# wsntxxn/AudioCaption

Measured on AMD Instinct MI355X. Metric: clips/sec (10 s @ 32 kHz) encode+greedy-decode, Cnn14_Rnn-Trm, higher is better.
Workload: dtype bf16x3

## Files before the change

audiocaption_amd/_lib.py:

```python
import ctypes
import os

import torch

_HERE = os.path.dirname(os.path.abspath(__file__))
LIB_PATH = os.environ.get("AUDIOCAPTION_HIP_LIB") or os.path.join(_HERE, "libaudiocaption_hip.so")

AC_MAX_LAYERS = 8
AC_ENS_MAX = 8
ABI_VERSION = 2

c_float_p = ctypes.c_void_p
c_int_p = ctypes.c_void_p


class AcTrmLayer(ctypes.Structure):
    _fields_ = [(n, ctypes.c_void_p) for n in (
        "sa_in_w", "sa_in_b", "sa_out_w", "sa_out_b", "ca_in_w", "ca_in_b", "ca_out_w", "ca_out_b",
        "l1_w", "l1_b", "l2_w", "l2_b", "n1_w", "n1_b", "n2_w", "n2_b", "n3_w", "n3_b")]


class AcTrmWeights(ctypes.Structure):
    _fields_ = [(n, ctypes.c_int32) for n in (
        "d_model", "nhead", "nlayers", "dim_ff", "vocab", "max_pos", "attn_emb_dim", "reserved")] + [
        (n, ctypes.c_void_p) for n in ("emb", "pe", "cls_w", "proj_w", "proj_b", "proj_ln_w", "proj_ln_b", "step_pk")] + [
        ("layer", AcTrmLayer * AC_MAX_LAYERS)]


class AcTrmKeyword(ctypes.Structure):
    _fields_ = [("kwp", ctypes.c_void_p), ("ln_w", ctypes.c_void_p), ("ln_b", ctypes.c_void_p), ("row_div", ctypes.c_int32)]


class AcLogitRules(ctypes.Structure):
    _fields_ = [("repetition_penalty", ctypes.c_float), ("no_repeat_ngram", ctypes.c_int32), ("min_length", ctypes.c_int32),
                ("end_idx", ctypes.c_int32), ("n_bad", ctypes.c_int32), ("bad_words", ctypes.c_void_p)]


class AcBahWeights(ctypes.Structure):
    _fields_ = [(n, ctypes.c_int32) for n in (
        "emb_dim", "d_model", "attn_size", "attn_emb_dim", "fc_emb_dim", "vocab", "n_tags", "variant")] + [
        (n, ctypes.c_void_p) for n in ("emb", "temb", "w_ih", "w_hh", "b_ih", "b_hh", "attn_w", "attn_b", "attn_v",
                                       "fc_w", "fc_b", "ctx_w", "ctx_b", "cls_w", "cls_b")]


class AcBahGrads(ctypes.Structure):
    _fields_ = [(n, ctypes.c_void_p) for n in ("emb", "temb", "w_ih", "w_hh", "b_ih", "b_hh", "attn_w", "attn_b", "attn_v",
                                               "fc_w", "fc_b", "ctx_w", "ctx_b", "cls_w", "cls_b")]


_I, _L, _F, _P = ctypes.c_int, ctypes.c_long, ctypes.c_float, ctypes.c_void_p
_U64 = ctypes.c_ulonglong
_WP = ctypes.POINTER(AcTrmWeights)
_BP = ctypes.c_void_p

SIGNATURES = {
    "ac_abi_version": (_I, []),
    "ac_logmel": (_I, [_P, _I, _I, _I, _I, _P, _P, _P, _P, _P, _P, _P, _P, _I, _L, _L, _L, _P]),
    "ac_conv3x3_bn_relu": (_I, [_P, _P, _P, _P, _P, _I, _I, _I, _I, _I, _I, _I, _I, _P]),
    "ac_conv3x3_bn_relu_winograd": (_I, [_P, _P, _P, _P, _P, _I, _I, _I, _I, _I, _I, _I, _I, _P]),
    "ac_conv3x3_bn_relu_bf16x3": (_I, [_P, _P, _P, _P, _P, _I, _I, _I, _I, _I, _I, _I, _I, _P]),
    "ac_conv3x3_bn_relu_bf16x3_gw": (_I, [_P, _P, _P, _P, _P, _I, _I, _I, _I, _I, _I, _I, _I, _P]),
    "ac_conv3x3_bn_relu_wino1d": (_I, [_P, _P, _P, _P, _P, _I, _I, _I, _I, _I, _I, _I, _I, _P, _I, _I, _P]),
    "ac_conv3x3_bn_relu_wino1d_drop": (_I, [_P, _P, _P, _P, _P, _I, _I, _I, _I, _I, _I, _I, _I, _F, _U64, _P, _P]),
    "ac_conv3x3_wino1d_splitk_floats": (_L, [_I, _I, _I, _I, _I]),
    "ac_conv3x3_bn_relu_wino1d_splitk": (_I, [_P, _P, _P, _P, _P, _I, _I, _I, _I, _I, _I, _I, _I, _P, _I, _I, _P, _L, _P]),
    "ac_conv3x3_bn_relu_wino43": (_I, [_P, _P, _P, _P, _P, _I, _I, _I, _I, _I, _I, _I, _I, _I, _P, _I, _I, _P]),
    "ac_conv3x3_bn_relu_wino43_drop": (_I, [_P, _P, _P, _P, _P, _I, _I, _I, _I, _I, _I, _I, _I, _F, _U64, _P, _P]),
    "ac_conv3x3_wino43_workgroups": (_L, [_I, _I, _I, _I]),
    "ac_conv3x3_block1_wino43": (_I, [_P, _P, _P, _P, _P, _P, _P, _P, _I, _I, _I, _P, _I, _I, _F, _U64, _P, _P]),
    "ac_conv3x3_block1_wino43_mfma": (_I, [_P, _P, _P, _P, _P, _P, _P, _P, _I, _I, _I, _P, _I, _I, _F, _U64, _P, _P]),
    "ac_conv3x3_block1_conv2_wino43": (_I, [_P, _P, _P, _P, _P, _I, _I, _I, _P]),
    "ac_conv3x3_bn_relu_f16x2_gw": (_I, [_P, _P, _P, _P, _P, _I, _I, _I, _I, _I, _I, _I, _I, _I, _P, _P]),
    "ac_conv3x3_block1_f16x2": (_I, [_P, _P, _P, _P, _P, _P, _P, _P, _I, _I, _I, _I, _P, _P]),
    "ac_linear_bf16x3": (_I, [_P, _P, _P, _P, _P, _I, _I, _I, _I, _P]),
    "ac_conv3x3_first": (_I, [_P, _P, _P, _P, _P, _I, _I, _I, _I, _P]),
    "ac_conv3x3_first_f16": (_I, [_P, _P, _P, _P, _P, _I, _I, _I, _I, _P, _P]),
    "ac_conv5x5_first": (_I, [_P, _P, _P, _P, _P, _I, _I, _I, _P]),
    "ac_conv5x5_bn_relu_bf16x3": (_I, [_P, _P, _P, _P, _P, _I, _I, _I, _I, _I, _I, _I, _P]),
    "ac_pack_conv5x5_weight_bf16x3": (_I, [_P, _P, _I, _I, _P]),
    "ac_linear": (_I, [_P, _P, _P, _P, _I, _I, _I, _L, _L, _L, _I, _P]),
    "ac_gru_pack_whh": (_I, [_P, _P, _I, _P]),
    "ac_gru_layer": (_I, [_P, _P, _P, _P, _P, _I, _I, _I, _P]),
    "ac_gru_split_workspace_bytes": (_L, [_I]),
    "ac_gru_layer_split": (_I, [_P, _P, _P, _P, _P, _P, _P, _I, _I, _I, _P]),
    "ac_mean_with_lens": (_I, [_P, _P, _P, _I, _I, _I, _I, _P]),
    "ac_add_layernorm": (_I, [_P, _P, _P, _P, _P, _I, _I, _L, _L, _L, _P]),
    "ac_trm_memory": (_I, [_WP, _P, _I, _I, _P, _P, _P]),
    "ac_trm_step_pack_floats": (_L, [_WP]),
    "ac_trm_pack_step_weights": (_I, [_WP, _P, _P]),
    "ac_dec_wide_packed_floats": (_L, [_I, _I]),
    "ac_dec_wide_pack": (_I, [_P, _L, _I, _I, _P, _P]),
    "ac_dec_wide_gemm": (_I, [_I, _P, _L, _P, _L, _P, _P, _P, _L, _I, _P, _P, _F, _P, _L, _P, _P, _P, _L, _I, _I, _I, _I, _I, _I, _P]),
    "ac_trm_workspace_floats": (_L, [_WP, _I, _I]),
    "ac_trm_greedy": (_I, [_WP, _P, _P, _I, _I, _I, _I, _I, _I, _P, _P, _P, _P, _P, _P, _P]),
    "ac_trm_greedy_segments": (_I, [_WP, _P, _P, _I, _I, _I, _I, _I, _I, _I, _P, _P, _P, _P, _P, _P, _P]),
    "ac_sample_rows": (_I, [_P, _L, _I, _I, _I, _I, _F, _F, _P, _I, _P, _P, _P]),
    "ac_trm_sample": (_I, [_WP, _P, _P, _I, _I, _I, _I, _I, _I, _P, _P, _P, _P, _P, _P, _I, _I, _F, _F, _P, _P]),
    "ac_trm_sample_multi": (_I, [_WP, _P, _P, _I, _I, _I, _I, _I, _I, _I, _P, _P, _P, _P, _P, _P, _I, _I, _F, _F, _P, _P]),
    "ac_conv3x3_skinny_workspace_floats": (_L, [_I, _I, _I, _I, _I]),
    "ac_conv3x3_bn_relu_skinny": (_I, [_P, _P, _P, _P, _P, _I, _I, _I, _I, _I, _I, _I, _P, _L, _F, _U64, _P, _P]),
    "ac_trm_cluster_pack_floats": (_L, [_WP]),
    "ac_trm_cluster_pack": (_I, [_WP, _P, _P]),
    "ac_trm_cluster_workspace_bytes": (_L, [_I]),
    "ac_trm_greedy_cluster": (_I, [_WP, _P, _P, _P, _I, _I, _I, _I, _I, _I, _P, _P, _P, _P, _P, _P, _I, _P]),
    "ac_trm_forward_tokens": (_I, [_WP, _P, _P, _I, _I, _P, _P, _I, _P, _P, _P, _P]),
    "ac_trm_beam_step": (_I, [_WP, _P, _P, _I, _I, _I, _I, _I, _F, _P, _P, _P, _P, _P, _P, _P]),
    "ac_trm_beam_update": (_I, [_P, _P, _P, _P, _P, _P, _P, _P, _P, _P, _P, _P, _I, _I, _I, _I, _I, _I, _I, _I, _P]),
    "ac_trm_beam_reorder": (_I, [_WP, _I, _I, _I, _P, _P, _P]),
    "ac_trm_beam_update_all": (_I, [_P, _P, _P, _P, _P, _P, _P, _P, _P, _P, _P, _P, _I, _I, _I, _I, _I, _I, _I, _I, _P]),
    "ac_trm_kw_greedy_segments": (_I, [_WP, _P, _P, _P, _I, _I, _I, _I, _I, _I, _I, _P, _P, _P, _P, _P, _P, _P]),
    "ac_trm_kw_sample": (_I, [_WP, _P, _P, _P, _I, _I, _I, _I, _I, _I, _P, _P, _P, _P, _P, _P, _I, _I, _F, _F, _P, _P]),
    "ac_trm_kw_forward_tokens": (_I, [_WP, _P, _P, _P, _I, _I, _P, _P, _I, _P, _P, _P, _P]),
    "ac_trm_kw_beam_step": (_I, [_WP, _P, _P, _P, _I, _I, _I, _I, _I, _F, _P, _P, _P, _P, _P, _P, _P]),
    "ac_trm_kw_embed_qkv": (_I, [_WP, _P, _I, _I, _I, _P, _L, _P, _P, _P]),
    "ac_trm_step_logits": (_I, [_WP, _P, _P, _I, _I, _I, _I, _I, _P, _P, _I, _P, _L, _P, _L, _P, _P]),
    "ac_ens_greedy_pick": (_I, [_P, _I, _L, _I, _I, _I, _I, _I, _I, _P, _P, _P, _P, _P, _P, _P]),
    "ac_ens_sample_pick": (_I, [_P, _I, _L, _I, _I, _I, _I, _F, _F, _P, _I, _I, _I, _I, _P, _P, _P, _P, _P, _P, _P, _P]),
    "ac_ens_beam_step_select": (_I, [_P, _I, _L, _I, _I, _I, _I, _F, _P, _P, _P, _P, _P]),
    "ac_group_beam_select": (_I, [_P, _L, _I, _I, _I, _I, _F, _F, _P, _P, _I, _L, _P, _P, _P, _P]),
    "ac_logit_rules_apply": (_I, [_P, _L, _P, _L, _I, _I, _P, _L, _I, _P, _P]),
    "ac_trm_search_rules": (_I, [_WP, _P, _P, _I, _I, _I, _I, _I, _I, _I, _P, _P, _P, _P, _P, _P, _I, _I, _F, _F, _P, _P, _P, _L,
                                 _P]),
    "ac_trm_beam_step_rules": (_I, [_WP, _P, _P, _I, _I, _I, _I, _I, _F, _P, _P, _P, _P, _P, _P, _P, _P, _P]),
    "ac_bah_workspace_floats": (_L, [_BP, _I, _I, _I, _I]),
    "ac_bah_memory": (_I, [_BP, _P, _P, _I, _I, _I, _I, _P, _P]),
    "ac_bah_memory_cond": (_I, [_BP, _P, _P, _I, _I, _I, _I, _P, _P]),
    "ac_bah_step_logits": (_I, [_BP, _P, _P, _I, _I, _I, _I, _I, _P, _P, _L, _P, _P, _P, _L, _P, _L, _P, _L, _L, _P, _P]),
    "ac_bah_greedy": (_I, [_BP, _P, _P, _P, _I, _I, _I, _I, _I, _I, _P, _P, _P, _P, _P, _P, _P, _P, _P]),
    "ac_bah_sample": (_I, [_BP, _P, _P, _P, _I, _I, _I, _I, _I, _I, _P, _P, _P, _P, _P, _P, _P, _P, _I, _I, _F, _F, _P, _P]),
    "ac_bah_beam_gather": (_I, [_P, _P, _P, _P, _P, _P, _P, _I, _I, _I, _I, _I, _I, _P]),
    "ac_bah_train_workspace_floats": (_L, [_BP, _I, _I, _I]),
    "ac_bah_train_forward": (_I, [_BP, _P, _P, _P, _P, _L, _P, _P, _I, _I, _I, _I, _F, _U64, _P, _P, _P, _P, _P, _P, _P, _P,
                                  _P]),
    "ac_bah_train_rollout": (_I, [_BP, _P, _P, _P, _P, _I, _I, _I, _I, _I, _F, _P, _P, _L, _F, _U64, _P, _P, _P, _P, _P, _P, _P,
                                  _P, _P, _P]),
    "ac_bah_train_backward": (_I, [_BP, _P, _P, _P, _P, _P, _I, _I, _I, _F, _U64, _P, _P, _P, _P, _P]),
    "ac_bah_train_forward_cond": (_I, [_BP, _P, _P, _P, _P, _L, _P, _I, _I, _I, _I, _F, _U64, _P, _P, _P, _P, _P, _P, _P, _P,
                                       _P]),
    "ac_bah_train_backward_cond": (_I, [_BP, _P, _P, _P, _P, _P, _I, _I, _I, _F, _U64, _P, _P, _P, _P, _P]),
    "ac_bah_mean_lens_bwd": (_I, [_P, _P, _P, _I, _I, _I, _I, _P]),
    "ac_specificity_loss": (_I, [_P, _P, _P, _P, _I, _I, _I, _I, _P, _P, _P, _P, _P]),
    "ac_specificity_loss_bwd": (_I, [_P, _P, _P, _P, _P, _P, _P, _I, _I, _I, _I, _P, _P]),
    "ac_pool_avgmax": (_I, [_P, _P, _I, _I, _I, _I, _I, _I, _I, _I, _P]),
    "ac_sed_head": (_I, [_P, _P, _P, _P, _L, _I, _P]),
    "ac_sed_tag_workspace_bytes": (_L, [_I, _I, _I]),
    "ac_sed_temporal_tag": (_I, [_P, _I, _I, _I, _I, _I, _F, _F, _I, _P, _P, _L, _P, _P]),
    "ac_gemm": (_I, [_P, _L, _L, _P, _L, _L, _P, _L, _I, _I, _I, _P, _I, _F, _I, _F, _U64, _P, _L, _P, _I, _P]),
    "ac_gemm_bf16x3": (_I, [_P, _L, _L, _P, _L, _L, _P, _L, _I, _I, _I, _P, _I, _F, _I, _F, _U64, _P, _L, _P, _I, _P]),
    "ac_dropout": (_I, [_P, _P, _L, _F, _U64, _P, _L, _P]),
    "ac_mask_pos_scale": (_I, [_P, _P, _L, _F, _P]),
    "ac_build_prefix": (_I, [_P, _I, _P, _I, _P, _I, _I, _P, _L, _I, _I, _P]),
    "ac_embed_fwd": (_I, [_P, _P, _P, _P, _P, _L, _L, _I, _F, _U64, _F, _U64, _P, _P]),
    "ac_embed_bwd": (_I, [_P, _P, _P, _L, _I, _F, _U64, _F, _U64, _P, _P]),
    "ac_kw_embed_fwd": (_I, [_P, _P, _P, _P, _P, _P, _P, _P, _P, _P, _L, _L, _I, _F, _U64, _F, _U64, _P, _F, _P]),
    "ac_kw_embed_bwd": (_I, [_P, _P, _P, _P, _P, _P, _P, _P, _P, _L, _I, _F, _U64, _F, _U64, _P, _F, _P]),
    "ac_dropadd_ln_fwd": (_I, [_P, _P, _P, _P, _P, _P, _L, _L, _L, _I, _F, _U64, _P, _F, _P]),
    "ac_dropadd_ln_bwd": (_I, [_P, _P, _P, _P, _P, _I, _P, _L, _P, _P, _L, _I, _F, _U64, _P, _F, _P]),
    "ac_attn_seq_fwd": (_I, [_P, _L, _P, _L, _P, _L, _P, _L, _P, _I, _I, _P, _P, _P, _P, _P, _P, _I, _I, _I, _I, _I,
                             _I, _I, _I, _F, _U64, _P, _P]),
    "ac_attn_seq_bwd": (_I, [_P, _L, _P, _L, _P, _L, _P, _I, _I, _P, _L, _P, _L, _P, _L, _P, _L, _P, _P, _P, _P, _I,
                             _I, _I, _I, _I, _I, _F, _U64, _P, _P]),
    "ac_attn_self_bwd_tiled": (_I, [_P, _L, _P, _L, _P, _L, _P, _I, _I, _P, _L, _P, _L, _P, _L, _P, _L, _P, _P, _P, _P,
                                    _I, _I, _I, _I, _I, _I, _F, _U64, _P, _P, _P]),
    "ac_gather_rows": (_I, [_P, _P, _P, _L, _I, _P]),
    "ac_scatter_add_rows": (_I, [_P, _P, _P, _L, _I, _P]),
    "ac_specaug": (_I, [_P, _P, _P, _I, _I, _I, _I, _I, _I, _P]),
    "ac_sum_replicas": (_I, [_P, _P, _L, _I, _P]),
    "ac_rows_mean_w": (_I, [_P, _P, _I, _I, _I, _I, _I, _P]),
    "ac_transpose": (_I, [_P, _P, _I, _I, _I, _P]),
    "ac_colsum": (_I, [_P, _L, _P, _L, _I, _P]),
    "ac_argmax_rows": (_I, [_P, _L, _I, _I, _P, _L, _P]),
    "ac_label_smoothing_loss": (_I, [_P, _P, _L, _P, _I, _I, _I, _F, _F, _P, _P, _P, _F, _P, _P]),
    "ac_scst_pick": (_I, [_P, _L, _I, _I, _F, _P, _I, _I, _P, _L, _P, _P, _P, _L, _P, _L, _P]),
    "ac_scst_loss": (_I, [_P, _P, _L, _P, _F, _I, _I, _I, _I, _P, _P, _P, _P, _P]),
    "ac_scst_group_reward": (_I, [_P, _I, _I, _I, _P, _P, _P]),
    "ac_kd_loss": (_I, [_P, _P, _P, _L, _P, _I, _I, _I, _F, _F, _F, _F, _P, _P, _P, _P, _F, _P, _P]),
    "ac_enc_kd_workspace_floats": (_L, [_I, _I]),
    "ac_enc_kd_loss": (_I, [_P, _L, _P, _L, _I, _I, _I, _P, _P, _P, _P, _P, _F, _P, _P, _P]),
    "ac_cider_workspace_bytes": (_L, [_L, _I, _I, _I]),
    "ac_cider_scores": (_I, [_P, _I, _L, _I, _I, _I, _I, _P, _I, _I, _P, _L, _P, _I, _I, _P, _I, _P, _P, _I, _F, _P, _L, _P,
                             _P, _P]),
    "ac_capmetrics_workspace_bytes": (_L, [_I, _I]),
    "ac_bleu_scores": (_I, [_P, _I, _L, _I, _I, _I, _I, _P, _I, _P, _L, _P, _I, _I, _P, _I, _P, _P, _I, _P, _L, _P, _P, _P,
                            _P]),
    "ac_rouge_l_scores": (_I, [_P, _I, _L, _I, _I, _I, _I, _P, _I, _P, _L, _P, _I, _I, _P, _I, _P, _P, _P, _L, _P, _P, _P,
                               _P]),
    "ac_diversity_workspace_bytes": (_L, [_I, _I]),
    "ac_diversity_scores": (_I, [_P, _L, _I, _I, _I, _I, _P, _I, _P, _L, _P, _P, _P, _P, _P, _P]),
    "ac_diversity_group_workspace_bytes": (_L, [_I, _I, _I]),
    "ac_diversity_group_scores": (_I, [_P, _L, _I, _I, _I, _I, _P, _I, _P, _I, _P, _L, _P, _P, _P, _P, _P, _P, _P, _P]),
    "ac_gru_layer_train": (_I, [_P, _P, _P, _P, _P, _P, _I, _I, _I, _P]),
    "ac_gru_layer_bwd": (_I, [_P, _P, _P, _P, _P, _P, _P, _P, _I, _I, _I, _P]),
    "ac_swa_update": (_I, [_P, _P, _L, _I, _P]),
    "ac_grad_sumsq": (_I, [_P, _L, _P, _P]),
    "ac_clip_coef": (_I, [_P, _F, _F, _P]),
    "ac_scale_by_coef": (_I, [_P, _L, _P, _P]),
    "ac_adam_step": (_I, [_P, _P, _P, _P, _L, _P, _F, _F, _F, _F, _F, _I, _P, _P]),
    "ac_adam_commit": (_I, [_P, _P, _P]),
    "ac_pointwise_conv": (_I, [_P, _P, _P, _P, _L, _I, _I, _I, _F, _P, _I, _P]),
    "ac_top_db_clamp": (_I, [_P, _L, _F, _P, _I, _P]),
    "ac_effnet_stem": (_I, [_P, _P, _P, _P, _P, _I, _I, _I, _I, _I, _I, _P]),
    "ac_effnet_depthwise": (_I, [_P, _P, _P, _P, _P, _P, _F, _I, _I, _I, _I, _I, _I, _I, _I, _P]),
    "ac_effnet_se_gate": (_I, [_P, _F, _P, _P, _P, _P, _P, _I, _I, _I, _P]),
    "ac_pw_gemm_packed_bytes": (_L, [_I, _I]),
    "ac_pw_gemm_pack": (_I, [_P, _P, _I, _I, _P]),
    "ac_pw_gemm_bf16x3": (_I, [_P, _P, _P, _P, _L, _I, _I, _I, _F, _P, _I, _P]),
    "ac_pw_gemm_bf16x3_ex": (_I, [_P, _L, _P, _P, _P, _L, _L, _I, _I, _I, _F, _P, _I, _F, _U64, _P, _L, _P]),
    "ac_pw_gemm_pack_strided": (_I, [_P, _L, _L, _P, _I, _I, _P]),
    "ac_pw_gemm_pack_table": (_I, [_P, _I, _P]),
    "ac_effnet_se_gate_t": (_I, [_P, _F, _P, _P, _P, _P, _P, _I, _I, _I, _P]),
    "ac_effnet_expand_depthwise": (_I, [_P, _P, _P, _P, _P, _P, _P, _P, _F, _I, _I, _I, _I, _I, _I, _I, _I, _I, _P]),
    "ac_ingest_resample": (_I, [_P, _I, _P, _P, _P, _P, _P, _P, _P, _I, _I, _I, _I, _I, _P]),
    "ac_htsat_patch_embed": (_I, [_P, _I, _I, _P, _P, _P, _P, _P, _I, _P]),
    "ac_swin_window_attn": (_I, [_P, _P, _P, _I, _I, _I, _I, _I, _I, _P]),
    "ac_swin_patch_merge": (_I, [_P, _P, _P, _P, _I, _I, _I, _I, _P]),
    "ac_htsat_pool": (_I, [_P, _P, _P, _I, _I, _I, _I, _I, _P]),
    "ac_htsat_token_mean": (_I, [_P, _P, _I, _I, _I, _P]),
    "ac_gelu": (_I, [_P, _P, _L, _P]),
    "ac_mfma_bf16_probe": (_I, [_P, _I, _I, _P]),
    "ac_placement_probe": (_I, [_P, _I, _I, _I, _P]),
    "ac_stream_create_cu_mask": (_I, [_I, _I, _P]),
    "ac_stream_destroy": (_I, [_P]),
}

_lib = None

PARAM_GENERATION = 0


_TENSOR_GENERATION = {}


def bump_param_generation(params=None):
    global PARAM_GENERATION
    import weakref
    PARAM_GENERATION += 1
    if params is not None:
        for p_ in params:
            hit = _TENSOR_GENERATION.get(id(p_))
            n = hit[1] + 1 if (hit is not None and hit[0]() is p_) else 1
            _TENSOR_GENERATION[id(p_)] = (weakref.ref(p_), n)


def param_generation():
    return PARAM_GENERATION


def tensor_generation(t):
    hit = _TENSOR_GENERATION.get(id(t))
    return hit[1] if (hit is not None and hit[0]() is t) else 0


def param_generation_flat(engine):
    return engine.flat.flat.data_ptr()


class HipLibraryError(RuntimeError):
    pass


def load():
    global _lib
    if _lib is not None:
        return _lib
    if not os.path.exists(LIB_PATH):
        raise HipLibraryError(
            f"{LIB_PATH} is missing: build it with `python -m audiocaption_amd.build` "
            "(hipcc --offload-arch=gfx950).  There is no CPU fallback on the product path.")
    lib = ctypes.CDLL(LIB_PATH)
    for name, (res, args) in SIGNATURES.items():
        fn = getattr(lib, name)
        fn.restype = res
        fn.argtypes = args
    if lib.ac_abi_version() != ABI_VERSION:
        raise HipLibraryError("libaudiocaption_hip.so ABI version mismatch; rebuild it")
    _lib = lib
    return lib


AC_ERR_ARG, AC_ERR_LAUNCH = -1, -2
_ERR = {-1: "AC_ERR_ARG (arguments rejected)", -2: "AC_ERR_LAUNCH (HIP launch failed)"}


def check(rc, what):
    if rc != 0:
        raise HipLibraryError(f"{what} failed: {_ERR.get(rc, rc)}")


def ptr(t):
    if t is None:
        return None
    if not t.is_cuda:
        raise HipLibraryError("the HIP path needs tensors on a ROCm device (got a CPU tensor); "
                              "there is no CPU fallback")
    return ctypes.c_void_p(t.data_ptr())


def stream():
    return ctypes.c_void_p(torch.cuda.current_stream().cuda_stream)


def f32c(t):
    if t.dtype != torch.float32:
        t = t.float()
    return t.contiguous()
```

audiocaption_amd/cnn_encoder.py:

```python
import dataclasses
import os
from typing import NamedTuple

import torch
import torch.nn as nn

from . import kernels as K
from .mel import MelSpectrogramBuffers, MelTables

CHANNELS = [1, 64, 128, 256, 512, 1024, 2048]


class ConvBlock(nn.Module):

    def __init__(self, in_channels, out_channels):
        super().__init__()
        self.conv1 = nn.Conv2d(in_channels, out_channels, (3, 3), (1, 1), (1, 1), bias=False)
        self.conv2 = nn.Conv2d(out_channels, out_channels, (3, 3), (1, 1), (1, 1), bias=False)
        self.bn1 = nn.BatchNorm2d(out_channels)
        self.bn2 = nn.BatchNorm2d(out_channels)
        for conv in (self.conv1, self.conv2):
            nn.init.xavier_uniform_(conv.weight)


def cnn14_feat_len(wav_len, hop, ratio=32):
    wav_len = torch.as_tensor(wav_len).cpu()
    n = torch.div(wav_len, hop, rounding_mode="floor") + 1
    return torch.div(n, ratio, rounding_mode="floor").long()


def wino1d_covers(cout):
    return cout % 128 == 0 or (cout == 64 and os.environ.get("AUDIOCAPTION_W1_C64", "1") != "0")


def _wino1d_clip_chunk(B, Hp, W, Cin):
    return max(1, min(B, ((1 << 31) - 1) // (W * Cin * 4 * Hp) - 1))


def _conv_wino1d(x, w, scale, shift, out, B, Hp, H, W, Cin, Cout, mode, need=None, dropout=None, workspace=None,
                 overflow=None, cold=False):
    if not wino1d_covers(Cout):
        K.conv3x3_bn_relu_bf16x3_gw(x, w, scale, shift, out, B, Hp, H, W, Cin, Cout, mode)
        if dropout is not None:
            K.dropout_(out, out.numel() if mode != 1 else B * (Hp // 2) * (W // 2) * Cout, *dropout)
        return out
    chunk = _wino1d_clip_chunk(B, Hp, W, Cin)
    if chunk < B:
        if dropout is not None:
            raise ValueError("F(2,3) conv: the dropout epilogue indexes the whole output buffer; batches beyond 2 GiB of input "
                             "are not supported in train mode")
        in_clip = Hp * W * Cin
        out_clip = {0: Hp * W * Cout, 1: (Hp // 2) * (W // 2) * Cout, 2: H * Cout}[mode]
        xf, of = x.reshape(-1), out.reshape(-1)
        for b0 in range(0, B, chunk):
            nb = min(chunk, B - b0)
            nd = (need[0][b0:b0 + nb], need[1], need[2]) if need is not None else None
            _conv_wino1d(xf[b0 * in_clip:(b0 + nb) * in_clip], w, scale, shift, of[b0 * out_clip:(b0 + nb) * out_clip], nb, Hp,
                         H, W, Cin, Cout, mode, need=nd, workspace=workspace)
        return out
    if dropout is not None:
        return K.conv3x3_bn_relu_wino1d(x, w, scale, shift, out, B, Hp, H, W, Cin, Cout, mode, dropout=dropout)
    ws = None
    if workspace is not None:
        floats = K.wino1d_splitk_floats(B, Hp, W, Cin, Cout)
        ws = workspace(floats) if floats else None
    return K.conv3x3_bn_relu_wino1d(x, w, scale, shift, out, B, Hp, H, W, Cin, Cout, mode, need=need, workspace=ws)


W43_MIN_WORKGROUPS = int(os.environ.get("AUDIOCAPTION_W43_MIN_WG", "192"))


def wino43_covers(W, cout):
    return W in (32, 16, 8, 4, 2) and cout % 128 == 0


class Wino43Pack(NamedTuple):
    f23: torch.Tensor
    f43: torch.Tensor = None
    skinny: "_LazyPack" = None


def _conv_wino43(x, w, scale, shift, out, B, Hp, H, W, Cin, Cout, mode, need=None, dropout=None, workspace=None,
                 overflow=None, cold=False):
    if w.f43 is not None and (mode != 1 if W == 2 else mode != 2) and Hp % 4 == 0 \
            and K.wino43_workgroups(B, Hp, W, Cout) >= W43_MIN_WORKGROUPS:
        return K.conv3x3_bn_relu_wino43(x, w.f43, scale, shift, out, B, Hp, H, W, Cin, Cout, mode, need=need, dropout=dropout)
    if w.skinny is not None and need is None and workspace is not None and SKINNY and (cold or dropout is not None) \
            and B * Hp * W <= SKINNY_MAX_PX:
        n = K.skinny_workspace_floats(B, Hp, W, Cin, Cout)
        if n > 0:
            return K.conv3x3_bn_relu_skinny(x, w.skinny.get(), scale, shift, out, B, Hp, H, W, Cin, Cout, mode, workspace(n),
                                            dropout=dropout)
    return _conv_wino1d(x, w.f23, scale, shift, out, B, Hp, H, W, Cin, Cout, mode, need=need, dropout=dropout,
                        workspace=workspace)


BLOCK1_CONV1 = os.environ.get("AUDIOCAPTION_BLOCK1_CONV1", "mfma")
SKINNY = os.environ.get("AUDIOCAPTION_SKINNY", "1") != "0"
SKINNY_MAX_PX = int(os.environ.get("AUDIOCAPTION_SKINNY_MAX_PX", "1024"))


class _LazyPack:

    def __init__(self, weight):
        self._weight, self._pk = weight, None

    def get(self):
        if self._pk is None:
            self._pk = K.pack_conv_weight_bf16x3_frag(self._weight.detach().float())
        return self._pk


def ragged_exact():
    return os.environ.get("AUDIOCAPTION_RAGGED_EXACT", "0") == "1"


def rows_needed(block, conv, quads=False):
    if block == 6:
        return (1, 0) if conv == 2 else (1, 1)
    if not quads:
        mul, add = 1 << (6 - block), (1 << (8 - block)) - 4
        return (mul, add) if conv == 2 else (mul, add + 1)
    need = 2 * 2
    mul = 2
    for b in range(5, block, -1):
        need = 2 * (need + 8)
        mul *= 2
    if block == 1:
        return (mul, need) if conv == 2 else (mul, need + 1)
    return (mul, need) if conv == 2 else (mul, need + 4)


@dataclasses.dataclass(frozen=True)
class ConvTier:
    pack: object
    launch: object
    act: torch.dtype = torch.float32
    block1: object = None
    pack_block1: object = None
    skips_dead_rows: bool = False
    f43: bool = False
    dropout_epilogue: bool = False
    overflow_word: bool = False
    fallback: str = None
    block6: str = None


def _plain(kernel, takes_overflow=False):
    def launch(x, w, scale, shift, out, B, Hp, H, W, Cin, Cout, mode, need=None, dropout=None, workspace=None, overflow=None,
               cold=False):
        if need is not None or dropout is not None:
            raise ValueError("this conv tier has neither dead-row skipping nor a dropout epilogue")
        if takes_overflow:
            return kernel(x, w, scale, shift, out, B, Hp, H, W, Cin, Cout, mode, overflow=overflow)
        return kernel(x, w, scale, shift, out, B, Hp, H, W, Cin, Cout, mode)
    return launch


def _pack_with(pack):
    return lambda w, b, weight: (pack(w), None)


def _pack_wino1d(w, b, weight):
    return (K.pack_conv_weight_wino1d_frag if wino1d_covers(w.shape[0]) else K.pack_conv_weight_bf16x3_frag)(w), None


def _pack_wino43(w, b, weight):
    return Wino43Pack(_pack_wino1d(w, b, weight)[0],
                      K.pack_conv_weight_wino43_frag(w) if wino43_covers(64 >> b, w.shape[0]) else None,
                      _LazyPack(weight) if b >= 4 else None), None


def _block1_wino43(x0, conv1, conv2, f43, out, B, Hp, H, need, dropout, overflow):
    if Hp % 8 != 0 or B * Hp // 8 < W43_MIN_WORKGROUPS:
        return False
    K.conv3x3_block1_wino43(x0, *conv1, f43, conv2[1], conv2[2], out, B, Hp, H, need=need, dropout=dropout,
                            conv1=BLOCK1_CONV1)
    return True


def _block1_f16x2(x0, conv1, conv2, pack, out, B, Hp, H, need, dropout, overflow):
    K.conv3x3_block1_f16x2(x0, *conv1, *conv2, out, B, Hp, H, 64, overflow=overflow)
    return True


TIERS = {
    "wino43": ConvTier(_pack_wino43, _conv_wino43, block1=_block1_wino43, pack_block1=K.pack_conv_weight_wino43_frag,
                       skips_dead_rows=True, f43=True, dropout_epilogue=True),
    "wino1d": ConvTier(_pack_wino1d, _conv_wino1d, skips_dead_rows=True, dropout_epilogue=True),
    "bf16x3": ConvTier(_pack_with(K.pack_conv_weight_bf16x3_frag), _plain(K.conv3x3_bn_relu_bf16x3_gw)),
    "bf16x3_lds": ConvTier(_pack_with(K.pack_conv_weight_bf16x3), _plain(K.conv3x3_bn_relu_bf16x3)),
    "f16x2": ConvTier(lambda w, b, weight: K.pack_conv_weight_f16x2_frag(w), _plain(K.conv3x3_bn_relu_f16x2_gw, True),
                      act=torch.float16, block1=_block1_f16x2, overflow_word=True, fallback="bf16x3", block6="bf16x3"),
    "winograd": ConvTier(_pack_with(K.pack_conv_weight_winograd), _plain(K.conv3x3_bn_relu_winograd)),
    "direct": ConvTier(_pack_with(K.pack_conv_weight), _plain(K.conv3x3_bn_relu)),
}


def conv_tier(algo):
    try:
        return TIERS[algo]
    except KeyError:
        raise ValueError(f"unknown conv_algo {algo!r}") from None


class _PannsEncoder(nn.Module):

    def _init_front(self, sample_rate):
        sr_to_fmax = {32000: 14000, 16000: 8000}
        self.sample_rate = sample_rate
        self.n_fft = 32 * sample_rate // 1000
        self.hop_length = 10 * sample_rate // 1000
        self.f_min, self.f_max = 50.0, float(sr_to_fmax[sample_rate])
        self.melspec_extractor = MelSpectrogramBuffers(sample_rate, self.n_fft, self.f_min, self.f_max, 64, "slaney",
                                                       "slaney")
        self.bn0 = nn.BatchNorm2d(64)
        self._tables = None
        self._tables_key = None
        self._packed = {}
        self._bufs = {}

    def _cached_pack(self, algo, layers, variant, build):
        tensors = [self.bn0.weight, self.bn0.bias, self.bn0.running_mean, self.bn0.running_var]
        for conv, bn in layers:
            tensors += [conv.weight, bn.weight, bn.bias, bn.running_mean, bn.running_var]
        key = tuple((t.data_ptr(), t._version, K._lib.tensor_generation(t)) for t in tensors) + (algo, variant)
        hit = self._packed.get(algo)
        if hit is not None and hit[0] == key:
            return hit[1]

        def fold(bn):
            return K.fold_bn(bn.weight.float(), bn.bias.float(), bn.running_mean.float(), bn.running_var.float(), bn.eps)

        with torch.no_grad():
            pk = build(fold)
        self._packed[algo] = (key, pk)
        return pk

    def _buf(self, name, numel, device, dtype=torch.float32):
        b = self._bufs.get((name, dtype))
        if b is None or b.numel() < numel or b.device != device:
            b = torch.empty(numel, device=device, dtype=dtype)
            self._bufs[(name, dtype)] = b
        return b

    def capture_token(self, algo):
        hit = self._packed.get(algo)
        ident = (id(hit[1]) if hit is not None else None,) + tuple(sorted((k[0], str(k[1]), b.data_ptr())
                                                                           for k, b in self._bufs.items()))
        return ident, (hit, dict(self._bufs), self._tables)

    def logmel_front(self, wav):
        dev = wav.device
        self._ensure_tables(dev)
        pk = self._pack(dev, self.effective_algo(None, False, None))
        Hp = self.geometry(wav.shape[1])[2]
        return K.logmel(wav, self._tables, pk["bn0"][0], pk["bn0"][1], rows_per_clip=Hp[0], channels_last=True)

    def _fc_emb(self, attn_emb, feat_length):
        lens = K.upload(feat_length, attn_emb.device, torch.int32)
        pooled = K.mean_with_lens(attn_emb, lens, add_max=True)
        return K.linear(pooled, self.fc1.weight.float(), self.fc1.bias.float(), relu=True)

    def _ensure_tables(self, dev):
        mkey = self.melspec_extractor.key()
        if self._tables is None or self._tables.window.device != dev or self._tables_key != mkey:
            self._tables = MelTables(self.sample_rate, self.n_fft, self.hop_length, self.f_min, self.f_max, 64,
                                     "slaney", "slaney", dev, window=self.melspec_extractor.spectrogram.window,
                                     fb=self.melspec_extractor.mel_scale.fb)
            self._tables_key = mkey


class Cnn14Encoder(_PannsEncoder):

    def __init__(self, sample_rate=32000, freeze=False):
        super().__init__()
        self._init_front(sample_rate)
        for b in range(6):
            setattr(self, f"conv_block{b + 1}", ConvBlock(CHANNELS[b], CHANNELS[b + 1]))
        self.downsample_ratio = 32
        self.fc1 = nn.Linear(2048, 2048, bias=True)
        nn.init.xavier_uniform_(self.fc1.weight)
        nn.init.zeros_(self.fc1.bias)
        self.fc_emb_size = 2048
        self.freeze = freeze
        self.conv_algo = os.environ.get("AUDIOCAPTION_CONV_ALGO", "wino43")
        self.f16x2_min_frames = int(os.environ.get("AUDIOCAPTION_F16X2_MIN_FRAMES", "10"))
        self.f16x2_block6 = os.environ.get("AUDIOCAPTION_F16X2_BLOCK6", "bf16x3")

    def load_pretrained(self, pretrained, output_fn=print):
        checkpoint = torch.load(pretrained, map_location="cpu")
        if "model" in checkpoint:
            sd = checkpoint["model"]
            if any(k.startswith("backbone.") for k in sd):
                sd = {k[len("backbone."):]: v for k, v in sd.items() if k.startswith("backbone.")}
        elif "state_dict" in checkpoint:
            sd = {k.replace("audio_encoder.", ""): v for k, v in checkpoint["state_dict"].items()
                  if "audio_encoder" in k}
        else:
            raise Exception("Unkown checkpoint format")
        own = self.state_dict()
        loaded = {k: v for k, v in sd.items() if k in own and own[k].shape == v.shape}
        output_fn(f"Loading pre-trained model, with mismatched keys {[k for k in sd if k not in loaded]}\n")
        own.update(loaded)
        self.load_state_dict(own, strict=True)
        if self.freeze:
            for name, param in self.named_parameters():
                param.requires_grad = name not in loaded

    def _pack(self, device, algo=None):
        algo = algo or self.conv_algo
        tier = conv_tier(algo)
        tier6 = conv_tier(tier.block6) if tier.block6 is not None and tier.block6 == self.f16x2_block6 else tier
        layers = [(b, conv, bn) for b, blk in enumerate(getattr(self, f"conv_block{b + 1}") for b in range(6))
                  for conv, bn in ((blk.conv1, blk.bn1), (blk.conv2, blk.bn2))]

        def build(fold):
            pk = {"bn0": fold(self.bn0), "convs": [], "block6": tier6, "block1": None}
            for i, (b, conv, bn) in enumerate(layers):
                w = conv.weight.detach().float()
                if i == 0:
                    wp, inv = w.reshape(64, 9).contiguous(), None
                else:
                    wp, inv = (tier6 if b == 5 else tier).pack(w, b, conv.weight)
                sc, sh = fold(bn)
                if inv is not None:
                    sc = (sc * inv).contiguous()
                pk["convs"].append((wp, sc, sh))
            if tier.pack_block1 is not None:
                pk["block1"] = tier.pack_block1(self.conv_block1.conv2.weight.detach().float())
            return pk

        return self._cached_pack(algo, [(conv, bn) for _, conv, bn in layers], tier6 is not tier, build)

    def geometry(self, n_samples):
        T = n_samples // self.hop_length + 1
        H = [T >> k for k in range(6)]
        if H[5] < 1:
            raise ValueError(f"clips of {n_samples} samples are shorter than one Cnn14 output frame")
        hp6 = (H[5] + 4) & ~3
        Hp = [hp6 << (5 - k) for k in range(6)]
        return T, H, Hp

    def encode(self, wav, dropout=None, specaug=None, train=False, min_frames=None, algo=None, overflow=None,
               clip_frames=None, x0=None, block6_f23=False):
        if wav.dim() != 2:
            raise ValueError("wav must be (batch, samples)")
        dev = wav.device
        self._ensure_tables(dev)
        algo = self.effective_algo(algo, train or dropout is not None, min_frames)
        pk = self._pack(dev, algo)
        B, L = wav.shape
        T, H, Hp = self.geometry(L)
        if x0 is None:
            x0 = K.logmel(wav, self._tables, pk["bn0"][0], pk["bn0"][1], rows_per_clip=Hp[0], channels_last=True)
        if specaug is not None:
            K.specaug_(x0, specaug, pk["bn0"][1], B, Hp[0], T)
        return self.conv_stack(x0, B, H, Hp, pk, algo, dropout, overflow=overflow, clip_frames=clip_frames,
                               block6_f23=block6_f23)

    def effective_algo(self, algo=None, train=False, min_frames=None):
        algo = algo or self.conv_algo
        fallback = conv_tier(algo).fallback
        if fallback is not None and (train or (min_frames is not None and min_frames < self.f16x2_min_frames)):
            return fallback
        return algo

    def conv_stack(self, x0, B, H, Hp, pk, algo, dropout=None, blocks=None, overflow=None, clip_frames=None,
                   block6_f23=False):
        dev = x0.device
        tiers = [conv_tier(algo)] * 5 + [pk["block6"]]
        full = self._buf("full", B * Hp[0] * 64 * 64, dev, tiers[0].act)
        pooled = self._buf("pooled", B * Hp[1] * 32 * 64, dev, tiers[0].act)
        W = 64
        offer = {"workspace": None, "overflow": overflow, "cold": dropout is not None}
        if os.environ.get("AUDIOCAPTION_W1_SPLITK", "1") != "0":
            offer["workspace"] = lambda n: self._buf("w1_splitk", n, dev)
        fuse1 = os.environ.get("AUDIOCAPTION_FUSE_BLOCK1", "1") != "0"
        for b in range(6):
            tier = tiers[b]
            cin, cout = CHANNELS[b], CHANNELS[b + 1]
            w1, s1, t1 = pk["convs"][2 * b]
            w2, s2, t2 = pk["convs"][2 * b + 1]
            if b == 5 and block6_f23 and tier.f43:
                w1, w2 = Wino43Pack(w1.f23), Wino43Pack(w2.f23)

            def need(j):
                if clip_frames is None or not tier.skips_dead_rows:
                    return None
                return (clip_frames,) + rows_needed(b + 1, j, quads=tier.f43 and ragged_exact())

            drop = (dropout[0], dropout[1] + b, dropout[2]) if dropout is not None else None
            epilogue = drop if tier.dropout_epilogue else None
            pool_out = pooled
            if b < 5 and tiers[b + 1].act != tier.act:
                pool_out = self._buf("pooled32", B * Hp[b + 1] * (W // 2) * cout, dev, tiers[b + 1].act)
            if tier.act != tiers[0].act:
                full = self._buf("full32", B * Hp[b] * W * cout, dev, tier.act)
            one_kernel = b == 0 and fuse1 and tier.block1 is not None \
                and tier.block1(x0, (w1, s1, t1), (w2, s2, t2), pk["block1"], pooled, B, Hp[0], H[0], need(2), epilogue, overflow)
            if b == 0 and not one_kernel:
                K.conv3x3_first(x0, w1, s1, t1, full, B, Hp[0], H[0], W, overflow=overflow)
            elif b > 0:
                tier.launch(pooled, w1, s1, t1, full, B, Hp[b], H[b], W, cin, cout, 0, need=need(1), **offer)
            if b < 5:
                if not one_kernel:
                    tier.launch(full, w2, s2, t2, pool_out, B, Hp[b], H[b], W, cout, cout, 1,
                                need=need(2) if epilogue is None else None, dropout=epilogue, **offer)
                pooled = pool_out
                W //= 2
                if drop is not None and epilogue is None:
                    K.dropout_(pooled, B * Hp[b + 1] * W * cout, *drop)
                if blocks is not None:
                    blk = pooled[:B * Hp[b + 1] * W * cout].reshape(B, Hp[b + 1], W, cout)[:, :H[b + 1]]
                    blocks.append(blk.permute(0, 3, 1, 2).float().clone())
            else:
                attn = torch.empty(B, H[5], cout, device=dev, dtype=torch.float32)
                if drop is None:
                    tier.launch(full, w2, s2, t2, attn, B, Hp[b], H[b], W, cout, cout, 2, need=need(2), **offer)
                else:
                    last = self._buf("last", B * Hp[5] * W * cout, dev)
                    tier.launch(full, w2, s2, t2, last, B, Hp[b], H[b], W, cout, cout, 0, dropout=epilogue, **offer)
                    if epilogue is None:
                        K.dropout_(last, B * Hp[5] * W * cout, *drop)
                    K.rows_mean_w(last, attn, B, Hp[5], H[5], W, cout)
        return attn

    def forward(self, input_dict, skip_fc=False):
        if self.training:
            raise NotImplementedError(
                "Cnn14Encoder (HIP path): in train mode the (frozen) Cnn14 only runs inside the whole-model training "
                "step (audiocaption_amd.train.TrainEngine); SpecAugment and the backward through the convolutions "
                "are not built")
        wav = input_dict["wav"]
        feat_length = cnn14_feat_len(input_dict["wav_len"], self.hop_length, self.downsample_ratio)
        min_frames = int(feat_length.min())
        algo = self.effective_algo(input_dict.get("conv_algo"), False, min_frames)
        tier = conv_tier(algo)
        flag = torch.zeros(1, device=wav.device, dtype=torch.int32) if tier.overflow_word else None
        ragged = skip_fc and tier.skips_dead_rows and os.environ.get("AUDIOCAPTION_SKIP_DEAD_ROWS", "1") != "0" \
            and int(feat_length.min()) < int(feat_length.max())
        frames = K.upload(feat_length, wav.device, torch.int32) if ragged else None
        uneven = skip_fc and ragged_exact() and int(feat_length.min()) < int(feat_length.max())
        attn_emb = self.encode(wav, min_frames=min_frames, algo=algo, overflow=flag, clip_frames=frames,
                               x0=input_dict.get("_logmel"), block6_f23=uneven)
        out = {"attn_emb": attn_emb, "attn_emb_len": feat_length}
        if flag is not None:
            out["f16_overflow"] = flag
        if not skip_fc:
            out["fc_emb"] = self._fc_emb(attn_emb, feat_length)
        return out


class ConvBlock5x5(nn.Module):

    def __init__(self, in_channels, out_channels):
        super().__init__()
        self.conv1 = nn.Conv2d(in_channels, out_channels, (5, 5), (1, 1), (2, 2), bias=False)
        self.bn1 = nn.BatchNorm2d(out_channels)
        nn.init.xavier_uniform_(self.conv1.weight)


class _CnnSmallEncoder(_PannsEncoder):
    block = None

    def __init__(self, sample_rate=32000, freeze=False):
        super().__init__()
        self._init_front(sample_rate)
        for b in range(4):
            setattr(self, f"conv_block{b + 1}", self.block(CHANNELS[b], CHANNELS[b + 1]))
        self.downsample_ratio = 16
        self.fc1 = nn.Linear(512, 512, bias=True)
        nn.init.xavier_uniform_(self.fc1.weight)
        nn.init.zeros_(self.fc1.bias)
        self.fc_emb_size = 512
        self.freeze = freeze

    def load_pretrained(self, pretrained, output_fn=print):
        from .config import merge_load_state_dict
        checkpoint = torch.load(pretrained, map_location="cpu")
        if "model" not in checkpoint:
            raise Exception("Unkown checkpoint format")
        loaded = merge_load_state_dict(checkpoint["model"], self, output_fn)
        if self.freeze:
            for name, param in self.named_parameters():
                param.requires_grad = name not in loaded

    def geometry(self, n_samples):
        T = n_samples // self.hop_length + 1
        H = [T >> k for k in range(5)]
        if H[4] < 1:
            raise ValueError(f"clips of {n_samples} samples ({T} frames) are shorter than one {type(self).__name__} output "
                             f"frame (16 frames)")
        hp4 = (H[4] + 3) & ~1
        return T, H, [hp4 << (4 - k) for k in range(5)]

    def _pack(self, device, algo=None):
        algo = self.effective_algo(algo)
        blocks = [getattr(self, f"conv_block{b + 1}") for b in range(4)]
        layers = [(b, getattr(blk, f"conv{j}"), getattr(blk, f"bn{j}")) for b, blk in enumerate(blocks)
                  for j in (1, 2) if hasattr(blk, f"conv{j}")]

        def build(fold):
            pk = {"bn0": fold(self.bn0), "convs": []}
            for i, (b, conv, bn) in enumerate(layers):
                w = conv.weight.detach().float()
                wp, inv = (w.reshape(64, -1).contiguous(), None) if i == 0 else self._pack_layer(algo, w, b, conv.weight)
                sc, sh = fold(bn)
                if inv is not None:
                    sc = (sc * inv).contiguous()
                pk["convs"].append((wp, sc, sh))
            self._pack_extra(algo, pk)
            return pk

        return self._cached_pack(algo, [(conv, bn) for _, conv, bn in layers], None, build)

    def _pack_extra(self, algo, pk):
        pass

    def encode(self, wav, algo=None, x0=None, blocks=None):
        if wav.dim() != 2:
            raise ValueError("wav must be (batch, samples)")
        dev = wav.device
        self._ensure_tables(dev)
        algo = self.effective_algo(algo)
        pk = self._pack(dev, algo)
        B, L = wav.shape
        T, H, Hp = self.geometry(L)
        if x0 is None:
            x0 = K.logmel(wav, self._tables, pk["bn0"][0], pk["bn0"][1], rows_per_clip=Hp[0], channels_last=True)
        return self.conv_stack(x0, B, H, Hp, pk, algo, blocks=blocks)

    def _head(self, pooled, B, H, Hp, blocks):
        attn = torch.empty(B, H[4], 512, device=pooled.device, dtype=torch.float32)
        return K.rows_mean_w(pooled, attn, B, Hp[4], H[4], 4, 512)

    @staticmethod
    def _keep(blocks, pooled, B, H, Hp, lvl, W, cout):
        if blocks is not None:
            blk = pooled[:B * Hp[lvl] * W * cout].reshape(B, Hp[lvl], W, cout)[:, :H[lvl]]
            blocks.append(blk.permute(0, 3, 1, 2).float().clone())

    def forward(self, input_dict, skip_fc=False):
        if self.training:
            name = type(self).__name__
            raise NotImplementedError(
                f"{name} (HIP path): inference only - call .eval(); the train-mode forward (SpecAugment, dropout) and the "
                f"backward through the convolutions are not built, and the whole-model training step "
                f"(audiocaption_amd.train.TrainEngine) trains over Cnn14Encoder only")
        wav = input_dict["wav"]
        algo = self.effective_algo(input_dict.get("conv_algo"))
        self.geometry(wav.shape[1])
        feat_length = cnn14_feat_len(input_dict["wav_len"], self.hop_length, self.downsample_ratio)
        attn_emb = self.encode(wav, algo=algo, x0=input_dict.get("_logmel"))
        out = {"attn_emb": attn_emb, "attn_emb_len": feat_length}
        if not skip_fc:
            out["fc_emb"] = self._fc_emb(attn_emb, feat_length)
        return out


class Cnn10Encoder(_CnnSmallEncoder):
    block = ConvBlock

    def __init__(self, sample_rate=32000, freeze=False):
        super().__init__(sample_rate, freeze)
        self.conv_algo = os.environ.get("AUDIOCAPTION_CONV_ALGO", "wino43")

    def effective_algo(self, algo=None, train=False, min_frames=None):
        algo = algo or self.conv_algo
        tier = conv_tier(algo)
        if tier.act != torch.float32:
            if tier.fallback is None:
                raise ValueError(f"conv tier {algo!r} keeps no f32 activations and declares no fallback")
            return tier.fallback
        return algo

    def _pack_layer(self, algo, w, b, weight):
        return conv_tier(algo).pack(w, b, weight)

    def _pack_extra(self, algo, pk):
        tier = conv_tier(algo)
        pk["block1"] = tier.pack_block1(self.conv_block1.conv2.weight.detach().float()) if tier.pack_block1 else None

    def conv_stack(self, x0, B, H, Hp, pk, algo, blocks=None):
        dev = x0.device
        tier = conv_tier(algo)
        full = self._buf("full", B * Hp[0] * 64 * 64, dev)
        pooled = self._buf("pooled", B * Hp[1] * 32 * 64, dev)
        offer = {"workspace": None}
        if os.environ.get("AUDIOCAPTION_W1_SPLITK", "1") != "0":
            offer["workspace"] = lambda n: self._buf("w1_splitk", n, dev)
        fuse1 = os.environ.get("AUDIOCAPTION_FUSE_BLOCK1", "1") != "0"
        W = 64
        for b in range(4):
            cin, cout = CHANNELS[b], CHANNELS[b + 1]
            conv1, conv2 = pk["convs"][2 * b], pk["convs"][2 * b + 1]
            one_kernel = b == 0 and fuse1 and tier.block1 is not None \
                and tier.block1(x0, conv1, conv2, pk["block1"], pooled, B, Hp[0], H[0], None, None, None)
            if b == 0 and not one_kernel:
                K.conv3x3_first(x0, *conv1, full, B, Hp[0], H[0], W)
            elif b > 0:
                tier.launch(pooled, *conv1, full, B, Hp[b], H[b], W, cin, cout, 0, **offer)
            if not one_kernel:
                tier.launch(full, *conv2, pooled, B, Hp[b], H[b], W, cout, cout, 1, **offer)
            W //= 2
            self._keep(blocks, pooled, B, H, Hp, b + 1, W, cout)
        return self._head(pooled, B, H, Hp, blocks)


class Cnn6Encoder(_CnnSmallEncoder):
    block = ConvBlock5x5
    conv_algo = "conv5x5"

    def effective_algo(self, algo=None, train=False, min_frames=None):
        if algo is not None and algo != self.conv_algo:
            raise ValueError(f"Cnn6Encoder runs on its own 5x5 kernels only (conv_algo {self.conv_algo!r}), not {algo!r}")
        return self.conv_algo

    def _pack_layer(self, algo, w, b, weight):
        return K.pack_conv5x5_weight(w), None

    def conv_stack(self, x0, B, H, Hp, pk, algo, blocks=None):
        dev = x0.device
        bufs = [self._buf("pooled", B * Hp[1] * 32 * 64, dev), self._buf("pooled_b", B * Hp[2] * 16 * 128, dev)]
        src = K.conv5x5_first(x0, *pk["convs"][0], bufs[0], B, Hp[0], H[0])
        self._keep(blocks, src, B, H, Hp, 1, 32, 64)
        W = 32
        for b in range(1, 4):
            cin, cout = CHANNELS[b], CHANNELS[b + 1]
            src = K.conv5x5_bn_relu_bf16x3(src, *pk["convs"][b], bufs[b & 1], B, Hp[b], H[b], W, cin, cout, 1)
            W //= 2
            self._keep(blocks, src, B, H, Hp, b + 1, W, cout)
        return self._head(src, B, H, Hp, blocks)


from .effnet_encoder import EfficientNetB2
```

audiocaption_amd/csrc/ac_wino43.h:

```cpp
#pragma once
#include "ac_common.h"

namespace {

typedef __bf16 bf16x8 __attribute__((ext_vector_type(8)));
typedef unsigned u32x2 __attribute__((ext_vector_type(2)));

__device__ __forceinline__ unsigned cvt_pk_bf16(float lo, float hi) {
  unsigned r;
  asm("v_cvt_pk_bf16_f32 %0, %1, %2" : "=v"(r) : "v"(lo), "v"(hi));
  return r;
}

__device__ __forceinline__ void split_bf16x4(const f32x4 x, u32x2& hi, u32x2& lo) {
  hi.x = cvt_pk_bf16(x[0], x[1]);
  hi.y = cvt_pk_bf16(x[2], x[3]);
  const float h0 = __builtin_bit_cast(float, hi.x << 16), h1 = __builtin_bit_cast(float, hi.x & 0xffff0000u);
  const float h2 = __builtin_bit_cast(float, hi.y << 16), h3 = __builtin_bit_cast(float, hi.y & 0xffff0000u);
  lo.x = cvt_pk_bf16(x[0] - h0, x[1] - h1);
  lo.y = cvt_pk_bf16(x[2] - h2, x[3] - h3);
}

__device__ __forceinline__ f32x4 vfma(float a, const f32x4 x, const f32x4 y) {
  f32x4 r;
#pragma unroll
  for (int j = 0; j < 4; ++j) r[j] = __builtin_fmaf(a, x[j], y[j]);
  return r;
}

__device__ __forceinline__ f32x4 w4_transform(int pos, const f32x4& d0, const f32x4& d1, const f32x4& d2, const f32x4& d3,
                                              const f32x4& d4, const f32x4& d5) {
  if (pos == 0) return vfma(4.f, d0, vfma(-5.f, d2, d4));
  if (pos == 5) return vfma(4.f, d1, vfma(-5.f, d3, d5));
  if (pos == 1 || pos == 2) {
    const f32x4 t1 = vfma(-4.f, d2, d4), t2 = vfma(-4.f, d1, d3);
    return pos == 1 ? t1 + t2 : t1 - t2;
  }
  const f32x4 t3 = d4 - d2, u = d3 - d1;
  return pos == 3 ? vfma(2.f, u, t3) : vfma(-2.f, u, t3);
}

__device__ __forceinline__ void w4_outputs(float m0, float m1, float m2, float m3, float m4, float m5, float sc, float sh,
                                           float (&y)[4]) {
  const float s12 = m1 + m2, d12 = m1 - m2, s34 = m3 + m4, d34 = m3 - m4;
  y[0] = fmaxf(fmaf((m0 + s12) + s34, sc, sh), 0.f);
  y[1] = fmaxf(fmaf(__builtin_fmaf(2.f, d34, d12), sc, sh), 0.f);
  y[2] = fmaxf(fmaf(__builtin_fmaf(4.f, s34, s12), sc, sh), 0.f);
  y[3] = fmaxf(fmaf(__builtin_fmaf(8.f, d34, d12) + m5, sc, sh), 0.f);
}

struct FastDiv4 {
  int d;
  float inv;
  __device__ __forceinline__ explicit FastDiv4(int d_) : d(d_), inv(1.0f / (float)d_) {}
  __device__ __forceinline__ int mod(int x) const {
    int q = (int)((float)x * inv);
    int r = x - q * d;
    if (r < 0) r += d;
    if (r >= d) r -= d;
    return r;
  }
};

__device__ __forceinline__ bool w4_rows_live(int row0, int nrows, int rows_total, int Hp, int H, const int* clip_frames,
                                             int need_mul, int need_add) {
  bool live = false;
  if (row0 < rows_total) {
    const int r_end = row0 + nrows < rows_total ? row0 + nrows : rows_total;
    int b = row0 / Hp;
    for (int base = b * Hp; base < r_end; base += Hp, ++b) {
      const int lo = (row0 > base ? row0 : base) - base;
      int lim = H;
      if (clip_frames) {
        const int need = need_mul * clip_frames[b] + need_add;
        lim = need < lim ? need : lim;
      }
      live = live || lo < lim;
    }
  }
  return live;
}

}
```

audiocaption_amd/csrc/conv3x3_wino43.hip:

```cpp
#include <stdlib.h>
#include <string.h>
#include <type_traits>

#include "ac_common.h"
#include "ac_drop.h"
#include "ac_wino43.h"

namespace {

#ifndef W4_KO
#define W4_KO 0
#endif

#ifndef W4_RING
#define W4_RING 9
#endif
#ifndef W4_PRO2
#define W4_PRO2 1
#endif
#ifndef W4_ADEPTH
#define W4_ADEPTH 2
#endif
#ifndef W4_ROWPAIR
#define W4_ROWPAIR 1
#endif

#ifdef W4_CLK
__device__ unsigned long long w4_clk[8];
#define W4_STAMP(var) const unsigned long long var = __builtin_readcyclecounter()
#else
#define W4_STAMP(var)
#endif

constexpr int KS = 16;
constexpr int W4_OUT_TILE = 4 * 32 * 144;

struct W4Params {
  const float* in;
  const void* wpk;
  const float* scale;
  const float* shift;
  float* out;
  int rows_total, Hp, H, W, Cin, Cout;
  int MT, NT;
  int Hp_out, H_out, W_out;
  int map_mode;
  const int* clip_frames;
  int need_mul, need_add;
  Drop drop;
};

enum { MODE_FULL = 0, MODE_POOL = 1, MODE_MEANW = 2 };

__device__ __forceinline__ bool w4_block_map(const W4Params& p, int& m_tile, int& n_tile) {
  const int bid = blockIdx.x;
  const int xcd = bid & 7, seq = bid >> 3;
  if (p.map_mode == 1) {
    n_tile = xcd + 8 * (seq / p.MT);
    m_tile = seq % p.MT;
  } else if (p.map_mode == 2) {
    n_tile = seq % p.NT;
    m_tile = (seq / p.NT) * 8 + xcd;
    if (m_tile >= p.MT) return false;
  } else if (p.map_mode == 3) {
    const int per = 8 / p.NT;
    n_tile = xcd % p.NT;
    m_tile = seq * per + xcd / p.NT;
    if (m_tile >= p.MT) return false;
  } else if (p.map_mode == 4) {
    const int per = 8 / p.NT;
    const int mtg = (p.MT + per - 1) / per;
    n_tile = xcd % p.NT;
    m_tile = (xcd / p.NT) * mtg + seq;
    if (seq >= mtg || m_tile >= p.MT) return false;
  } else {
    n_tile = bid % p.NT;
    m_tile = bid / p.NT;
  }
  return true;
}

template <int TC, int MW>
struct W4Geom {
  static_assert(TC == 32 || TC == 16 || TC == 8 || TC == 4 || TC == 2, "full-width blocks of 32, 16, 8, 4 or 2 mel columns");
  static_assert(MW == 1 || MW == 2, "one or two MFMA tiles per wave");
  static constexpr bool COLT = TC == 2;
  static_assert(!COLT || MW == 2, "column tiles: one tile per column");
  static constexpr int QT = COLT ? 32 : 32 / TC;
  static constexpr int PQ = COLT ? 32 : MW * QT;
  static constexpr int LCOLS = COLT ? 2 : TC + 2;
  static constexpr int COLP = COLT ? 32 : TC == 32 ? (PQ | 1) : TC == 16 ? (PQ % 4 == 2 ? PQ : PQ + 2) : (PQ % 8 == 4 ? PQ : PQ + 4);
  static constexpr int HALF = ((LCOLS * COLP * 16 + 127) / 128) * 128 + 64;
  static constexpr int PLANE = 2 * HALF;
  static constexpr int VBUF = 12 * PLANE;
  static constexpr int NITEM = PQ * TC * 4;
  static_assert(NITEM == 256 || NITEM == 128, "one item per thread (MW = 1: per thread of waves 0 and 1)");
  static constexpr int NPIECE = 6;
};

template <int MODE, int TC, int MW>
__global__ __launch_bounds__(256, MW == 1 ? 2 : 1) void conv3x3_w4_kernel(W4Params p) {
  using G = W4Geom<TC, MW>;
  constexpr int QT = G::QT, PQ = G::PQ, COLP = G::COLP, HALF = G::HALF, PLANE = G::PLANE, VBUF = G::VBUF;
  constexpr int NPIECE = G::NPIECE;
  extern __shared__ __attribute__((aligned(128))) unsigned char dsm_raw[];
  const int tid = threadIdx.x;
  const int lane = tid & 63;
  const int wave = __builtin_amdgcn_readfirstlane(tid >> 6);
  const int half = lane >> 5;

  int m_tile, n_tile;
  if (!w4_block_map(p, m_tile, n_tile)) return;
  W4_STAMP(clk_t0);
#ifdef W4_CLK
  const unsigned long long clk_rt0 = __builtin_amdgcn_s_memrealtime();
  unsigned long long clk_t1 = clk_t0;
#endif
  const int quad0 = m_tile * PQ;
  unsigned char* sV = dsm_raw;

  unsigned pb[MW];
  {
    const int i = lane & 31;
#pragma unroll
    for (int m = 0; m < MW; ++m)
      pb[m] = G::COLT ? (unsigned)(half * HALF + (m * COLP + i) * 16)
                      : (unsigned)(half * HALF + ((i % TC) * COLP + m * QT + i / TC) * 16);
  }

  f32x16 acc[6][MW];
#pragma unroll
  for (int q = 0; q < 6; ++q)
#pragma unroll
    for (int m = 0; m < MW; ++m)
#pragma unroll
      for (int r = 0; r < 16; ++r) acc[q][m][r] = 0.f;

  const int row0 = 4 * quad0;
  const bool live = w4_rows_live(row0, 4 * PQ, p.rows_total, p.Hp, p.H, p.clip_frames, p.need_mul, p.need_add);
  const bool all_pad = !live;
  const int nstep = p.Cin / KS;
  if (!all_pad) {
    const int R0 = row0 > 0 ? row0 - 1 : 0;
    const int first = row0 > 0 ? 0 : 1;
    const size_t row_elems = (size_t)p.W * p.Cin;
    const size_t left = ((size_t)p.rows_total - R0) * row_elems * 4;
    const __amdgpu_buffer_rsrc_t rin = __builtin_amdgcn_make_buffer_rsrc(
        (void*)(p.in + (size_t)R0 * row_elems), 0, (int)(left < 0x7fffffffull ? left : 0x7fffffffull), 0x00020000);
    const int NT32 = p.Cout >> 5;
    const unsigned g_bytes = (unsigned)NT32 * 2048u;
    const __amdgpu_buffer_rsrc_t rw = __builtin_amdgcn_make_buffer_rsrc(
        (void*)p.wpk, 0, (int)((unsigned)nstep * 18u * g_bytes), 0x00020000);
    const unsigned wvoff = (unsigned)((n_tile * 4 + wave) * 2048 + lane * 16);
    auto w_load = [&](int s, int gi, bf16x8 (&w)[2]) {
      if (W4_KO & 1) { if (s | gi) return; }
      const unsigned soff = (unsigned)(s * 18 + gi) * g_bytes;
      w[0] = __builtin_bit_cast(bf16x8, __builtin_amdgcn_raw_buffer_load_b128(rw, wvoff, soff, 0));
      w[1] = __builtin_bit_cast(bf16x8, __builtin_amdgcn_raw_buffer_load_b128(rw, wvoff + 1024u, soff, 0));
    };

    const unsigned row_bytes = (unsigned)row_elems * 4u;
    const bool stager = tid < G::NITEM;
    unsigned vbA, lofsA;
    {
      auto item = [&](int it, unsigned& vb, unsigned& lofs) {
        const int cq = it & 3, rest = it >> 2, quad = rest % PQ, c = rest / PQ;
        vb = (unsigned)(((4 * quad - first) * p.W + c) * p.Cin * 4 + cq * 16);
        lofs = (unsigned)((cq >> 1) * HALF + ((c + (G::COLT ? 0 : 1)) * COLP + quad) * 16 + (cq & 1) * 8);
      };
      item(stager ? tid : 0, vbA, lofsA);
    }

    auto run = [&]() {
      constexpr bool PAIR = W4_ROWPAIR && MW == 2;
      static_assert(!PAIR || W4_PRO2, "the paired form starts from the two-step prologue");
      f32x4 preA[6], rwp[PAIR ? 6 : 1];
      auto rows_request_pair = [&](int s) {
        if (W4_KO & 8) { if (s > 1) return; }
        const unsigned cs = (unsigned)(s * KS * 4);
#pragma unroll
        for (int r = 0; r < 6; ++r) {
          preA[r] = __builtin_bit_cast(f32x4, __builtin_amdgcn_raw_buffer_load_b128(rin, vbA + cs + (unsigned)r * row_bytes, 0, 0));
          rwp[PAIR ? r : 0] = __builtin_bit_cast(f32x4, __builtin_amdgcn_raw_buffer_load_b128(rin, vbA + cs + (unsigned)(KS * 4) + (unsigned)r * row_bytes, 0, 0));
        }
      };
      auto rows_request = [&](int s) {
        if (W4_KO & 8) { if (s) return; }
        if (!stager) return;
        const unsigned cs = (unsigned)(s * KS * 4);
#pragma unroll
        for (int r = 0; r < 6; ++r)
          preA[r] = __builtin_bit_cast(f32x4, __builtin_amdgcn_raw_buffer_load_b128(rin, vbA + cs + (unsigned)r * row_bytes, 0, 0));
      };
      auto store_piece = [&](unsigned char* buf, unsigned lofs, int pos, const f32x4 v) {
        u32x2 hi, lo;
        split_bf16x4(v, hi, lo);
        unsigned char* dst = buf + lofs + (2 * pos) * PLANE;
        *(u32x2*)dst = hi;
        *(u32x2*)(dst + PLANE) = lo;
      };
      auto commit_piece_set1 = [&](unsigned char* buf, int k) {
        if (W4_KO & 4) return;
        store_piece(buf, lofsA, k, w4_transform(k, rwp[0], rwp[PAIR ? 1 : 0], rwp[PAIR ? 2 : 0], rwp[PAIR ? 3 : 0],
                                                rwp[PAIR ? 4 : 0], rwp[PAIR ? 5 : 0]));
      };
      auto commit_piece = [&](unsigned char* buf, int k) {
        if (W4_KO & 4) return;
        if (!stager) return;
        store_piece(buf, lofsA, k, w4_transform(k, preA[0], preA[1], preA[2], preA[3], preA[4], preA[5]));
      };
      auto tap_valid = [](int m, int kx) { return !G::COLT || (m + kx - 1 >= 0 && m + kx - 1 <= 1); };
      auto a_load = [&](const unsigned char* buf, int gi, bf16x8 (&a)[MW][2]) {
        if (W4_KO & 2) { if (gi) return; }
        const int kx = gi / 6, q = gi % 6;
        const unsigned char* vh = buf + (2 * q) * PLANE;
        const int koff = (G::COLT ? kx - 1 : kx) * COLP * 16;
#pragma unroll
        for (int m = 0; m < MW; ++m) {
          if (!tap_valid(m, kx)) continue;
          a[m][0] = *(const bf16x8*)(vh + ((int)pb[m] + koff));
          a[m][1] = *(const bf16x8*)(vh + PLANE + ((int)pb[m] + koff));
        }
      };

      {
        constexpr int NZ = G::COLT ? 0 : 2 * 12 * 2 * 2 * COLP;
        const f32x4 z = {0.f, 0.f, 0.f, 0.f};
        for (int i = tid; i < NZ; i += 256) {
          const int slot = i % COLP, col = (i / COLP) & 1, hh = (i / (2 * COLP)) % 24, b = i / (48 * COLP);
          *(f32x4*)(sV + b * VBUF + hh * HALF + ((col ? TC + 1 : 0) * COLP + slot) * 16) = z;
        }
      }
      constexpr int RING = MW == 1 ? 6 : W4_RING, AH = RING - 1, NA = W4_ADEPTH + 1, LASTG = 17 - W4_ADEPTH;
      static_assert(18 % RING == 0 && 18 % NA == 0 && NPIECE <= LASTG, "ring positions are static; staging ends before the barrier");
      bf16x8 wr[RING][2];
#if W4_PRO2
      f32x4 pre2[6];
      if (PAIR) rows_request_pair(0);
      else rows_request(0);
      if (MW == 2 && !PAIR) {
        const unsigned cs = (unsigned)(KS * 4);
#pragma unroll
        for (int r = 0; r < 6; ++r)
          pre2[r] = __builtin_bit_cast(f32x4, __builtin_amdgcn_raw_buffer_load_b128(rin, vbA + cs + (unsigned)r * row_bytes, 0, 0));
      }
#pragma unroll
      for (int g0 = 0; g0 < AH; ++g0) w_load(0, g0, wr[g0]);
#pragma unroll
      for (int k = 0; k < NPIECE; ++k) commit_piece(sV, k);
      if (PAIR) {
      } else if (MW == 2) {
#pragma unroll
        for (int r = 0; r < 6; ++r) preA[r] = pre2[r];
      } else {
        rows_request(1);
      }
#else
#pragma unroll
      for (int g0 = 0; g0 < AH; ++g0) w_load(0, g0, wr[g0]);
      rows_request(0);
#pragma unroll
      for (int k = 0; k < NPIECE; ++k) commit_piece(sV, k);
      rows_request(1);
#endif
      lds_barrier();
      bf16x8 af[NA][MW][2];
#pragma unroll
      for (int g0 = 0; g0 < W4_ADEPTH; ++g0) a_load(sV, g0, af[g0]);

      auto step = [&](int s, auto MORE_, auto ODD_) {
        constexpr bool MORE = decltype(MORE_)::value;
        constexpr bool ODD = decltype(ODD_)::value;
        const unsigned char* cur = sV + (s & 1) * VBUF;
        unsigned char* nxt = sV + ((s + 1) & 1) * VBUF;
#pragma unroll
        for (int gi = 0; gi < 18; ++gi) {
          const int q = gi % 6;
          if (gi + W4_ADEPTH < 18) a_load(cur, gi + W4_ADEPTH, af[(gi + W4_ADEPTH) % NA]);
          else if (MORE) a_load(nxt, gi + W4_ADEPTH - 18, af[(gi + W4_ADEPTH) % NA]);
          if (gi + AH < 18) w_load(s, gi + AH, wr[(gi + AH) % RING]);
          else if (MORE) w_load(s + 1, gi + AH - 18, wr[(gi + AH) % RING]);
          if (!(W4_KO & 32)) {
            const int kxg = gi / 6;
#pragma unroll
            for (int m = 0; m < MW; ++m)
              if (tap_valid(m, kxg))
                acc[q][m] = __builtin_amdgcn_mfma_f32_32x32x16_bf16(wr[gi % RING][0], af[gi % NA][m][1], acc[q][m], 0, 0, 0);
#pragma unroll
            for (int m = 0; m < MW; ++m)
              if (tap_valid(m, kxg))
                acc[q][m] = __builtin_amdgcn_mfma_f32_32x32x16_bf16(wr[gi % RING][1], af[gi % NA][m][0], acc[q][m], 0, 0, 0);
#pragma unroll
            for (int m = 0; m < MW; ++m)
              if (tap_valid(m, kxg))
                acc[q][m] = __builtin_amdgcn_mfma_f32_32x32x16_bf16(wr[gi % RING][0], af[gi % NA][m][0], acc[q][m], 0, 0, 0);
          } else {
#pragma unroll
            for (int m = 0; m < MW; ++m)
              if (tap_valid(m, gi / 6))
                asm volatile("" :: "v"(af[gi % NA][m][0]), "v"(af[gi % NA][m][1]), "v"(wr[gi % RING][0]), "v"(wr[gi % RING][1]));
          }
          if (MORE) {
            if (PAIR) {
              if (gi < NPIECE) { if (ODD) commit_piece(nxt, gi); else commit_piece_set1(nxt, gi); }
              if (gi == NPIECE && !ODD) rows_request_pair(s + 2);
            } else {
              if (gi < NPIECE) commit_piece(nxt, gi);
              if (gi == NPIECE) rows_request(s + 2);
            }
          }
          if (gi == LASTG && !(W4_KO & 16)) lds_barrier();
          __builtin_amdgcn_sched_barrier(0);
        }
      };
#ifdef W4_CLK
      clk_t1 = __builtin_readcyclecounter();
#endif
      if (PAIR) {
#pragma unroll 1
        for (int s = 0; s + 2 < nstep; s += 2) {
          step(s, std::true_type{}, std::false_type{});
          step(s + 1, std::true_type{}, std::true_type{});
        }
        step(nstep - 2, std::true_type{}, std::false_type{});
        step(nstep - 1, std::false_type{}, std::true_type{});
      } else {
#pragma unroll 1
        for (int s = 0; s + 1 < nstep; ++s) step(s, std::true_type{}, std::false_type{});
        step(nstep - 1, std::false_type{}, std::false_type{});
      }
    };
    run();
  }

  W4_STAMP(clk_t2);
  const int chw = n_tile * 128 + wave * 32 + 4 * half;
  const FastDiv4 by_hp(p.Hp), by_hp_out(MODE == MODE_POOL ? p.Hp_out : 1);
  const int pi = lane & 31;
  const f32x4 zero4 = {0.f, 0.f, 0.f, 0.f};
  f32x4 sc4[4], sh4[4];
#pragma unroll
  for (int g = 0; g < 4; ++g) {
    sc4[g] = all_pad ? zero4 : *(const f32x4*)(p.scale + chw + 8 * g);
    sh4[g] = all_pad ? zero4 : *(const f32x4*)(p.shift + chw + 8 * g);
  }
  if (MODE == MODE_MEANW) {
    static_assert(MODE != MODE_MEANW || G::COLT, "the mean over mel is the two-column form's epilogue");
    const int qg = quad0 + pi, gr = 4 * qg;
    const int bclip = gr / p.Hp, h = gr - bclip * p.Hp;
#pragma unroll
    for (int g = 0; g < 4; ++g) {
      f32x4 mean[4];
#pragma unroll
      for (int e = 0; e < 4; ++e) {
        const int r = 4 * g + e;
        float ya[4], yb[4];
        w4_outputs(acc[0][0][r], acc[1][0][r], acc[2][0][r], acc[3][0][r], acc[4][0][r], acc[5][0][r], sc4[g][e], sh4[g][e], ya);
        w4_outputs(acc[0][1][r], acc[1][1][r], acc[2][1][r], acc[3][1][r], acc[4][1][r], acc[5][1][r], sc4[g][e], sh4[g][e], yb);
#pragma unroll
        for (int j = 0; j < 4; ++j) mean[j][e] = 0.5f * (ya[j] + yb[j]);
      }
      if (gr < p.rows_total) {
#pragma unroll
        for (int j = 0; j < 4; ++j)
          if (h + j < p.H && !(W4_KO & 64)) *(f32x4*)(p.out + ((size_t)bclip * p.H + h + j) * p.Cout + chw + 8 * g) = mean[j];
      }
    }
  } else {
#pragma unroll
  for (int m = 0; m < MW; ++m) {
    const int col = G::COLT ? m : pi % TC;
    const int qg = quad0 + (G::COLT ? pi : m * QT + pi / TC);
    const int gr = 4 * qg;
    f32x4 y[4][4];
#pragma unroll
    for (int g = 0; g < 4; ++g)
#pragma unroll
      for (int e = 0; e < 4; ++e) {
        const int r = 4 * g + e;
        float yy[4];
        w4_outputs(acc[0][m][r], acc[1][m][r], acc[2][m][r], acc[3][m][r], acc[4][m][r], acc[5][m][r], sc4[g][e], sh4[g][e], yy);
#pragma unroll
        for (int j = 0; j < 4; ++j) y[g][j][e] = yy[j];
      }
    unsigned char* wt = dsm_raw + wave * W4_OUT_TILE;
    constexpr int PITCH = 144;
    const int P8 = lane >> 3, q8 = lane & 7;
    if (MODE == MODE_FULL) {
      const int h = by_hp.mod(gr);
#pragma unroll
      for (int j = 0; j < 4; ++j)
#pragma unroll
        for (int g = 0; g < 4; ++g)
          *(f32x4*)(wt + (j * 32 + pi) * PITCH + (2 * g + half) * 16) = h + j < p.H ? y[g][j] : zero4;
#pragma unroll
      for (int k = 0; k < 4; ++k) {
        const int px = 8 * k + P8;
        const int pcol = G::COLT ? m : px % TC;
        const int pgr = 4 * (quad0 + (G::COLT ? px : m * QT + px / TC));
#pragma unroll
        for (int j = 0; j < 4; ++j) {
          f32x4 v = *(const f32x4*)(wt + (j * 32 + px) * PITCH + q8 * 16);
          const size_t oi = ((size_t)(pgr + j) * p.W + pcol) * p.Cout + n_tile * 128 + wave * 32 + 4 * q8;
          if (p.drop.thresh != 0) {
#pragma unroll
            for (int e = 0; e < 4; ++e) v[e] *= p.drop.mask(oi + e);
          }
          if (pgr < p.rows_total && !(W4_KO & 64)) *(f32x4*)(p.out + oi) = v;
        }
      }
    } else {
      const bool valid = by_hp_out.mod(2 * qg) + (col & 1) < p.H_out;
#pragma unroll
      for (int g = 0; g < 4; ++g) {
        const f32x4 t0 = y[g][0] + y[g][1], t1 = y[g][2] + y[g][3];
        f32x4 o;
#pragma unroll
        for (int e = 0; e < 4; ++e) {
          const float a = t0[e] + dpp_mov<DPP_QUAD_XOR1>(t0[e]), b = t1[e] + dpp_mov<DPP_QUAD_XOR1>(t1[e]);
          o[e] = 0.25f * ((col & 1) ? b : a);
        }
        *(f32x4*)(wt + pi * PITCH + (2 * g + half) * 16) = valid ? o : zero4;
      }
#pragma unroll
      for (int k = 0; k < 4; ++k) {
        const int px = 8 * k + P8;
        const int pcol = px % TC, pqg = quad0 + m * QT + px / TC;
        f32x4 o = *(const f32x4*)(wt + px * PITCH + q8 * 16);
        const size_t oi = ((size_t)(2 * pqg + (pcol & 1)) * p.W_out + (pcol >> 1)) * p.Cout + n_tile * 128 + wave * 32 + 4 * q8;
        if (p.drop.thresh != 0) {
#pragma unroll
          for (int e = 0; e < 4; ++e) o[e] *= p.drop.mask(oi + e);
        }
        if (4 * pqg < p.rows_total && !(W4_KO & 64)) *(f32x4*)(p.out + oi) = o;
      }
    }
  }
  }
#ifdef W4_CLK
  __builtin_amdgcn_s_waitcnt(0);
  if (tid == 0) {
    const unsigned long long t3 = __builtin_readcyclecounter();
    atomicAdd(&w4_clk[0], clk_t1 - clk_t0);
    atomicAdd(&w4_clk[1], clk_t2 - clk_t1);
    atomicAdd(&w4_clk[2], t3 - clk_t2);
    atomicAdd(&w4_clk[3], __builtin_amdgcn_s_memrealtime() - clk_rt0);
    atomicAdd(&w4_clk[4], 1ull);
  }
#endif
}

template <int MODE, int TC, int MW>
int launch_w4(W4Params p, hipStream_t s) {
  using G = W4Geom<TC, MW>;
  const int quads = p.rows_total / 4;
  p.MT = (quads + G::PQ - 1) / G::PQ;
  unsigned grid;
  if (p.map_mode == 2) grid = (unsigned)(((p.MT + 7) / 8) * 8 * p.NT);
  else if (p.map_mode == 3 || p.map_mode == 4) grid = (unsigned)(((p.MT + 8 / p.NT - 1) / (8 / p.NT)) * 8);
  else grid = (unsigned)(p.MT * p.NT);
  constexpr size_t lds = (size_t)2 * G::VBUF > (size_t)4 * W4_OUT_TILE ? (size_t)2 * G::VBUF : (size_t)4 * W4_OUT_TILE;
  static_assert(lds <= 160 * 1024, "V planes exceed the LDS");
  static AcLdsAttr lds_attr;
  if (ac_allow_lds((const void*)conv3x3_w4_kernel<MODE, TC, MW>, 160 * 1024, &lds_attr) != AC_OK) return AC_ERR_LAUNCH;
  hipLaunchKernelGGL((conv3x3_w4_kernel<MODE, TC, MW>), dim3(grid), dim3(256), lds, s, p);
  return ac_check_launch();
}

template <int MODE, int TC>
int launch_w4_mw(const W4Params& p, int mw, hipStream_t s) {
  if (mw == 1) return launch_w4<MODE, TC, 1>(p, s);
  return launch_w4<MODE, TC, 2>(p, s);
}

}

static long w4_grid(int rows_total, int W, int Cout, int mw) {
  const int pq = W == 2 ? 32 : mw * (32 / W);
  return (long)((rows_total / 4 + pq - 1) / pq) * (Cout / 128);
}

static int w4_dispatch(const float* in, const void* wfrag, const float* scale, const float* shift, float* out, int B, int Hp,
                       int H, int W, int Cin, int Cout, int mode, int map_mode, int mw, const int* clip_frames, int need_mul,
                       int need_add, void* stream, Drop drop) {
  if (!in || !wfrag || !scale || !shift || !out) return AC_ERR_ARG;
  if (B <= 0 || Hp <= H || (Hp & 3) || !(W == 32 || W == 16 || W == 8 || W == 4 || W == 2) || Cin % 32 || Cin < 32 || Cout % 128)
    return AC_ERR_ARG;
  if (W == 2 ? (mode != MODE_FULL && mode != MODE_MEANW) : (mode != MODE_FULL && mode != MODE_POOL)) return AC_ERR_ARG;
  if (mode == MODE_MEANW && drop.thresh != 0) return AC_ERR_ARG;
  if ((unsigned long long)B * Hp >= (1ull << 23)) return AC_ERR_ARG;
  if ((unsigned long long)(Cin / 16) * 18 * (Cout / 32) * 2048 >= (1ull << 31)) return AC_ERR_ARG;
  W4Params p;
  p.in = in; p.wpk = wfrag; p.scale = scale; p.shift = shift; p.out = out;
  p.rows_total = B * Hp; p.Hp = Hp; p.H = H; p.W = W; p.Cin = Cin; p.Cout = Cout;
  p.MT = 0;
  p.NT = Cout / 128;
  p.Hp_out = Hp / 2; p.H_out = H / 2; p.W_out = W / 2;
#ifndef W4_MW1_STEPS
#define W4_MW1_STEPS 4
#endif
#ifndef W4_DEFAULT_MAP
#define W4_DEFAULT_MAP 4
#endif
  if (map_mode < 0) map_mode = (p.NT % 8 == 0 && p.NT > 8) ? 1 : ((p.NT == 1 || p.NT == 2 || p.NT == 4 || p.NT == 8) ? W4_DEFAULT_MAP : 2);
  if (map_mode == 1 && p.NT % 8 != 0) return AC_ERR_ARG;
  if ((map_mode == 3 || map_mode == 4) && !(p.NT == 1 || p.NT == 2 || p.NT == 4 || p.NT == 8)) return AC_ERR_ARG;
  if (map_mode > 4) return AC_ERR_ARG;
  p.map_mode = map_mode;
  p.clip_frames = clip_frames; p.need_mul = need_mul; p.need_add = need_add;
  p.drop = drop;
  if (mw != 1 && mw != 2) {
    static const int mw1_max_steps = getenv("AUDIOCAPTION_W4_MW1_STEPS") ? atoi(getenv("AUDIOCAPTION_W4_MW1_STEPS")) : W4_MW1_STEPS;
    mw = (W != 2 && Cin / KS <= mw1_max_steps) ? 1 : 2;
  }
  if (W == 2) mw = 2;
  hipStream_t s = (hipStream_t)stream;
#define W4_CASE(TCV)                                                                     \
  if (W == TCV) return mode == MODE_FULL ? launch_w4_mw<MODE_FULL, TCV>(p, mw, s) : launch_w4_mw<MODE_POOL, TCV>(p, mw, s);
  W4_CASE(32) W4_CASE(16) W4_CASE(8) W4_CASE(4)
#undef W4_CASE
  if (W == 2) return mode == MODE_FULL ? launch_w4<MODE_FULL, 2, 2>(p, s) : launch_w4<MODE_MEANW, 2, 2>(p, s);
  return AC_ERR_ARG;
}

#ifdef W4_CLK
extern "C" int ac_w4_clk_read(unsigned long long* out5, int reset) {
  if (hipMemcpyFromSymbol(out5, HIP_SYMBOL(w4_clk), 40) != hipSuccess) return -2;
  if (reset) { unsigned long long z[8] = {0, 0, 0, 0, 0, 0, 0, 0}; if (hipMemcpyToSymbol(HIP_SYMBOL(w4_clk), z, 64) != hipSuccess) return -2; }
  return 0;
}
#endif

extern "C" int ac_conv3x3_bn_relu_wino43(const float* in, const void* wfrag, const float* scale, const float* shift,
                                         float* out, int B, int Hp, int H, int W, int Cin, int Cout, int mode,
                                         int map_mode, int tiles_per_wave, const int* clip_frames, int need_mul,
                                         int need_add, void* stream) {
  return w4_dispatch(in, wfrag, scale, shift, out, B, Hp, H, W, Cin, Cout, mode, map_mode, tiles_per_wave, clip_frames,
                     need_mul, need_add, stream, make_drop(0.f, 0, nullptr));
}

extern "C" int ac_conv3x3_bn_relu_wino43_drop(const float* in, const void* wfrag, const float* scale, const float* shift,
                                              float* out, int B, int Hp, int H, int W, int Cin, int Cout, int mode,
                                              int map_mode, float drop_p, unsigned long long drop_seed,
                                              const unsigned long long* seed_dev, void* stream) {
  if (!(drop_p >= 0.f) || drop_p >= 1.f) return AC_ERR_ARG;
  return w4_dispatch(in, wfrag, scale, shift, out, B, Hp, H, W, Cin, Cout, mode, map_mode, 0, nullptr, 0, 0, stream,
                     make_drop(drop_p, drop_seed, seed_dev));
}

extern "C" long ac_conv3x3_wino43_workgroups(int B, int Hp, int W, int Cout) {
  if (B <= 0 || Hp <= 0 || (Hp & 3) || !(W == 32 || W == 16 || W == 8 || W == 4 || W == 2) || Cout % 128) return 0;
  return w4_grid(B * Hp, W, Cout, 2);
}
```

audiocaption_amd/kernels.py:

```python
import contextlib
import ctypes
import os

import torch

from . import _lib
from ._lib import check, f32c, ptr, stream


def upload(t, device, dtype=None):
    t = torch.as_tensor(t)
    if t.is_cuda:
        return t.to(device=device, dtype=dtype)
    if dtype is not None:
        t = t.to(dtype)
    pin = torch.empty(t.shape, dtype=t.dtype, pin_memory=True)
    pin.copy_(t)
    return pin.to(device, non_blocking=True)


def _dev(t):
    if not t.is_cuda:
        raise _lib.HipLibraryError("the HIP path needs tensors on a ROCm device; there is no CPU fallback")
    return t


def logmel(wav, tables, scale=None, shift=None, rows_per_clip=None, channels_last=True):
    lib = _lib.load()
    wav = f32c(_dev(wav))
    B, L = wav.shape
    T = L // tables.hop + 1
    if channels_last:
        Hp = rows_per_clip if rows_per_clip is not None else T
        out = torch.empty(B * Hp, 64, device=wav.device, dtype=torch.float32)
        sb, st, sm = Hp * 64, 64, 1
    else:
        Hp = T
        out = torch.empty(B, 64, T, device=wav.device, dtype=torch.float32)
        sb, st, sm = 64 * T, 1, T
    check(lib.ac_logmel(ptr(wav), B, L, tables.n_fft, tables.hop, ptr(tables.window), ptr(tables.twiddle),
                        ptr(tables.melfb), ptr(tables.mel_lo), ptr(tables.mel_hi), ptr(scale), ptr(shift),
                        ptr(out), Hp, sb, st, sm, stream()), "ac_logmel")
    return out


def conv3x3_first(x, w, scale, shift, out, B, Hp, H, W=64, overflow=None):
    lib = _lib.load()
    if out.dtype == torch.float16:
        check(lib.ac_conv3x3_first_f16(ptr(x), ptr(w), ptr(scale), ptr(shift), ptr(out), B, Hp, H, W, ptr(overflow),
                                       stream()), "ac_conv3x3_first_f16")
        return out
    check(lib.ac_conv3x3_first(ptr(x), ptr(w), ptr(scale), ptr(shift), ptr(out), B, Hp, H, W, stream()),
          "ac_conv3x3_first")
    return out


def conv3x3_block1_f16x2(x0, w1, scale1, shift1, wfrag2, scale2, shift2, out, B, Hp, H, W=64, overflow=None):
    lib = _lib.load()
    if out.dtype != torch.float16:
        raise ValueError("conv3x3_block1_f16x2 writes fp16")
    check(lib.ac_conv3x3_block1_f16x2(ptr(x0), ptr(w1), ptr(scale1), ptr(shift1), ptr(wfrag2), ptr(scale2),
                                      ptr(shift2), ptr(out), B, Hp, H, W, ptr(overflow), stream()),
          "ac_conv3x3_block1_f16x2")
    return out


CONV_LAUNCH_HOOK = None


class _Observed:

    def __init__(self, hook, info):
        self.hook, self.info = hook, info

    def __enter__(self):
        self.hook("pre", self.info)

    def __exit__(self, *exc):
        self.hook("post", self.info)


_UNOBSERVED = contextlib.nullcontext()


def _observed(algo, B, Hp, H, W, Cin, Cout, mode, **more):
    hook = CONV_LAUNCH_HOOK
    if hook is None:
        return _UNOBSERVED
    return _Observed(hook, dict(B=B, H=H, Hp=Hp, W=W, Cin=Cin, Cout=Cout, mode=mode, algo=algo, **more))


def conv3x3_bn_relu(x, wpk, scale, shift, out, B, Hp, H, W, Cin, Cout, mode, map_mode=-1):
    lib = _lib.load()
    with _observed("direct", B, Hp, H, W, Cin, Cout, mode):
        check(lib.ac_conv3x3_bn_relu(ptr(x), ptr(wpk), ptr(scale), ptr(shift), ptr(out), B, Hp, H, W, Cin, Cout,
                                     mode, map_mode, stream()), "ac_conv3x3_bn_relu")
    return out


def conv3x3_bn_relu_winograd(x, upk, scale, shift, out, B, Hp, H, W, Cin, Cout, mode, map_mode=-1):
    lib = _lib.load()
    with _observed("winograd", B, Hp, H, W, Cin, Cout, mode):
        check(lib.ac_conv3x3_bn_relu_winograd(ptr(x), ptr(upk), ptr(scale), ptr(shift), ptr(out), B, Hp, H, W, Cin, Cout,
                                              mode, map_mode, stream()), "ac_conv3x3_bn_relu_winograd")
    return out


def conv3x3_bn_relu_bf16x3(x, wpk, scale, shift, out, B, Hp, H, W, Cin, Cout, mode, map_mode=-1):
    lib = _lib.load()
    with _observed("bf16x3", B, Hp, H, W, Cin, Cout, mode):
        check(lib.ac_conv3x3_bn_relu_bf16x3(ptr(x), ptr(wpk), ptr(scale), ptr(shift), ptr(out), B, Hp, H, W, Cin, Cout,
                                            mode, map_mode, stream()), "ac_conv3x3_bn_relu_bf16x3")
    return out


def pack_conv_weight_bf16x3(w):
    cout, cin = w.shape[0], w.shape[1]
    hi = w.to(torch.bfloat16)
    lo = (w - hi.float()).to(torch.bfloat16)

    def lay(t):
        return t.permute(1, 2, 3, 0).reshape(cin // 32, 32, 9, cout).permute(0, 2, 3, 1)

    return torch.stack([lay(hi), lay(lo)], dim=2).contiguous()


def conv3x3_bn_relu_bf16x3_gw(x, wfrag, scale, shift, out, B, Hp, H, W, Cin, Cout, mode, map_mode=-1):
    lib = _lib.load()
    with _observed("bf16x3", B, Hp, H, W, Cin, Cout, mode):
        check(lib.ac_conv3x3_bn_relu_bf16x3_gw(ptr(x), ptr(wfrag), ptr(scale), ptr(shift), ptr(out), B, Hp, H, W, Cin, Cout,
                                               mode, map_mode, stream()), "ac_conv3x3_bn_relu_bf16x3_gw")
    return out


def conv5x5_first(x, w, scale, shift, out, B, Hp, H):
    check(_lib.load().ac_conv5x5_first(ptr(x), ptr(w), ptr(scale), ptr(shift), ptr(out), B, Hp, H, stream()),
          "ac_conv5x5_first")
    return out


def conv5x5_bn_relu_bf16x3(x, wfrag, scale, shift, out, B, Hp, H, W, Cin, Cout, mode):
    with _observed("conv5x5", B, Hp, H, W, Cin, Cout, mode):
        check(_lib.load().ac_conv5x5_bn_relu_bf16x3(ptr(x), ptr(wfrag), ptr(scale), ptr(shift), ptr(out), B, Hp, H, W, Cin,
                                                    Cout, mode, stream()), "ac_conv5x5_bn_relu_bf16x3")
    return out


def pack_conv5x5_weight(w):
    cout, cin = w.shape[0], w.shape[1]
    if tuple(w.shape[2:]) != (5, 5):
        raise ValueError("pack_conv5x5_weight: OIHW with a 5x5 kernel")
    w = f32c(_dev(w))
    out = torch.empty(cin // 32, 25, 2, cout // 32, 2, 64, 8, device=w.device, dtype=torch.bfloat16)
    check(_lib.load().ac_pack_conv5x5_weight_bf16x3(ptr(w), ptr(out), cin, cout, stream()), "ac_pack_conv5x5_weight_bf16x3")
    return out


def wino1d_splitk_floats(B, Hp, W, Cin, Cout):
    return int(_lib.load().ac_conv3x3_wino1d_splitk_floats(B, Hp, W, Cin, Cout))


def conv3x3_bn_relu_wino1d(x, wfrag, scale, shift, out, B, Hp, H, W, Cin, Cout, mode, map_mode=-1, need=None,
                           workspace=None, dropout=None):
    lib = _lib.load()
    cf, mul, add = need if need is not None else (None, 0, 0)
    if dropout is not None and cf is not None:
        raise ValueError("conv3x3_bn_relu_wino1d: dropout and dead-row skipping are not combined")
    with _observed("wino1d", B, Hp, H, W, Cin, Cout, mode):
        if dropout is not None:
            check(lib.ac_conv3x3_bn_relu_wino1d_drop(ptr(x), ptr(wfrag), ptr(scale), ptr(shift), ptr(out), B, Hp, H, W, Cin,
                                                     Cout, mode, map_mode, float(dropout[0]), int(dropout[1]), dropout[2],
                                                     stream()), "ac_conv3x3_bn_relu_wino1d_drop")
        elif workspace is not None:
            check(lib.ac_conv3x3_bn_relu_wino1d_splitk(ptr(x), ptr(wfrag), ptr(scale), ptr(shift), ptr(out), B, Hp, H, W, Cin,
                                                       Cout, mode, map_mode, ptr(cf), int(mul), int(add), ptr(workspace),
                                                       workspace.numel(), stream()), "ac_conv3x3_bn_relu_wino1d_splitk")
        else:
            check(lib.ac_conv3x3_bn_relu_wino1d(ptr(x), ptr(wfrag), ptr(scale), ptr(shift), ptr(out), B, Hp, H, W, Cin,
                                                Cout, mode, map_mode, ptr(cf), int(mul), int(add), stream()),
                  "ac_conv3x3_bn_relu_wino1d")
    return out


def conv3x3_block1_wino43(x0, w1, scale1, shift1, wfrag2, scale2, shift2, out, B, Hp, H, need=None, dropout=None,
                          conv1="mfma"):
    if conv1 not in ("mfma", "valu"):
        raise ValueError(f"conv1 = {conv1!r}")
    cf, mul, add = need if need is not None else (None, 0, 0)
    dp, dseed, ddev = dropout if dropout is not None else (0.0, 0, None)
    name = "ac_conv3x3_block1_wino43_mfma" if conv1 == "mfma" else "ac_conv3x3_block1_wino43"
    with _observed("block1_w4", B, Hp, H, 64, 1, 64, 1, conv1=conv1):
        check(getattr(_lib.load(), name)(ptr(x0), ptr(w1), ptr(scale1), ptr(shift1), ptr(wfrag2), ptr(scale2), ptr(shift2),
                                         ptr(out), B, Hp, H, ptr(cf), int(mul), int(add), float(dp), int(dseed), ddev,
                                         stream()), name)
    return out


def conv3x3_block1_conv2_wino43(x64, wfrag2, scale2, shift2, out, B, Hp, H):
    check(_lib.load().ac_conv3x3_block1_conv2_wino43(ptr(x64), ptr(wfrag2), ptr(scale2), ptr(shift2), ptr(out), B, Hp, H,
                                                     stream()), "ac_conv3x3_block1_conv2_wino43")
    return out


def wino43_workgroups(B, Hp, W, Cout):
    return int(_lib.load().ac_conv3x3_wino43_workgroups(B, Hp, W, Cout))


def conv3x3_bn_relu_wino43(x, wfrag, scale, shift, out, B, Hp, H, W, Cin, Cout, mode, map_mode=-1, need=None, dropout=None,
                           tiles_per_wave=0):
    lib = _lib.load()
    cf, mul, add = need if need is not None else (None, 0, 0)
    if dropout is not None and cf is not None:
        raise ValueError("conv3x3_bn_relu_wino43: dropout and dead-row skipping are not combined")
    with _observed("wino43", B, Hp, H, W, Cin, Cout, mode):
        if dropout is not None:
            check(lib.ac_conv3x3_bn_relu_wino43_drop(ptr(x), ptr(wfrag), ptr(scale), ptr(shift), ptr(out), B, Hp, H, W, Cin,
                                                     Cout, mode, map_mode, float(dropout[0]), int(dropout[1]), dropout[2],
                                                     stream()), "ac_conv3x3_bn_relu_wino43_drop")
        else:
            check(lib.ac_conv3x3_bn_relu_wino43(ptr(x), ptr(wfrag), ptr(scale), ptr(shift), ptr(out), B, Hp, H, W, Cin, Cout,
                                                mode, map_mode, int(tiles_per_wave), ptr(cf), int(mul), int(add), stream()),
                  "ac_conv3x3_bn_relu_wino43")
    return out


def skinny_workspace_floats(B, Hp, W, Cin, Cout):
    return int(_lib.load().ac_conv3x3_skinny_workspace_floats(B, Hp, W, Cin, Cout))


def conv3x3_bn_relu_skinny(x, wfrag, scale, shift, out, B, Hp, H, W, Cin, Cout, mode, workspace, dropout=None):
    dp, dseed, ddev = dropout if dropout is not None else (0.0, 0, None)
    with _observed("skinny", B, Hp, H, W, Cin, Cout, mode):
        check(_lib.load().ac_conv3x3_bn_relu_skinny(ptr(x), ptr(wfrag), ptr(scale), ptr(shift), ptr(out), B, Hp, H, W, Cin, Cout,
                                                   mode, ptr(workspace), workspace.numel(), float(dp), int(dseed), ddev, stream()),
              "ac_conv3x3_bn_relu_skinny")
    return out


def conv3x3_bn_relu_f16x2_gw(x, wfrag, scale, shift, out, B, Hp, H, W, Cin, Cout, mode, map_mode=-1, overflow=None):
    lib = _lib.load()
    out_f32 = 1 if (mode == 1 and out.dtype == torch.float32) else 0
    if x.dtype != torch.float16 or out.dtype != (torch.float32 if (mode == 2 or out_f32) else torch.float16):
        raise ValueError("f16x2 conv: fp16 activations in, fp16 out (f32 for mode 2)")
    with _observed("f16x2", B, Hp, H, W, Cin, Cout, mode):
        check(lib.ac_conv3x3_bn_relu_f16x2_gw(ptr(x), ptr(wfrag), ptr(scale), ptr(shift), ptr(out), B, Hp, H, W,
                                              Cin, Cout, mode, map_mode, out_f32, ptr(overflow), stream()),
              "ac_conv3x3_bn_relu_f16x2_gw")
    return out


def pack_conv_weight_f16x2_frag(w):
    cout, cin = w.shape[0], w.shape[1]
    amax = w.abs().amax(dim=(1, 2, 3)).clamp_min(1e-30)
    e = 13 - torch.floor(torch.log2(amax))
    ws = w * torch.exp2(e).view(-1, 1, 1, 1)
    hi = ws.to(torch.float16)
    lo = (ws - hi.float()).to(torch.float16)

    def lay(t):
        t = t.permute(1, 2, 3, 0).reshape(cin // 32, 2, 2, 8, 9, cout // 32, 32)
        return t.permute(0, 4, 1, 5, 2, 6, 3).reshape(cin // 32, 9, 2, cout // 32, 64, 8)

    return torch.stack([lay(hi), lay(lo)], dim=4).contiguous(), torch.exp2(-e).contiguous()


def pack_conv_weight_bf16x3_frag(w):
    cout, cin = w.shape[0], w.shape[1]
    hi = w.to(torch.bfloat16)
    lo = (w - hi.float()).to(torch.bfloat16)

    taps = w.shape[2] * w.shape[3]

    def lay(t):
        t = t.permute(1, 2, 3, 0).reshape(cin // 32, 2, 2, 8, taps, cout // 32, 32)
        return t.permute(0, 4, 1, 5, 2, 6, 3).reshape(cin // 32, taps, 2, cout // 32, 64, 8)

    return torch.stack([lay(hi), lay(lo)], dim=4).contiguous()


def pack_conv_weight_wino1d_frag(w):
    cout, cin = w.shape[0], w.shape[1]
    g = w.double()
    u = torch.stack([g[:, :, 0], 0.5 * (g[:, :, 0] + g[:, :, 1] + g[:, :, 2]),
                     0.5 * (g[:, :, 0] - g[:, :, 1] + g[:, :, 2]), g[:, :, 2]], dim=3)
    u = u.reshape(cout, cin, 12, 1)
    hi = u.to(torch.bfloat16)
    lo = (u - hi.double()).to(torch.bfloat16)

    def lay(t):
        t = t.permute(1, 2, 3, 0).reshape(cin // 32, 2, 2, 8, 12, cout // 32, 32)
        return t.permute(0, 4, 1, 5, 2, 6, 3).reshape(cin // 32, 12, 2, cout // 32, 64, 8)

    return torch.stack([lay(hi), lay(lo)], dim=4).contiguous()


def pack_conv_weight_wino43_frag(w):
    cout, cin = w.shape[0], w.shape[1]
    g = w.double()
    G = ((1 / 4, 0, 0), (-1 / 6, -1 / 6, -1 / 6), (-1 / 6, 1 / 6, -1 / 6), (1 / 24, 1 / 12, 1 / 6), (1 / 24, -1 / 12, 1 / 6),
         (0, 0, 1))
    u = torch.stack([G[p][0] * g[:, :, 0] + G[p][1] * g[:, :, 1] + G[p][2] * g[:, :, 2] for p in range(6)], dim=3)
    u = u.reshape(cout, cin, 18)
    hi = u.to(torch.bfloat16)
    lo = (u - hi.double()).to(torch.bfloat16)

    def lay(t):
        t = t.permute(1, 2, 0).reshape(cin // 16, 2, 8, 18, cout // 32, 32)
        return t.permute(0, 3, 4, 1, 5, 2).reshape(cin // 16, 18, cout // 32, 64, 8)

    return torch.stack([lay(hi), lay(lo)], dim=3).contiguous()


def pack_conv_weight_winograd(w):
    cout, cin = w.shape[0], w.shape[1]

    def g_times(t, dim):
        t0, t1, t2 = t.select(dim, 0), t.select(dim, 1), t.select(dim, 2)
        return torch.stack([t0, 0.5 * (t0 + t1 + t2), 0.5 * (t0 - t1 + t2), t2], dim=dim)

    out = torch.empty(cin // 32, 4, 4, cout, 32, device=w.device, dtype=torch.float32)
    step = max(1, (1 << 22) // (cin * 16))
    for o0 in range(0, cout, step):
        u = g_times(g_times(w[o0:o0 + step].double(), 2), 3)
        u = u.permute(1, 3, 2, 0).reshape(cin // 32, 32, 4, 4, -1).permute(0, 2, 3, 4, 1)
        out[:, :, :, o0:o0 + step] = u.float()
    return out


def pack_conv_weight(w):
    cout, cin = w.shape[0], w.shape[1]
    return (w.permute(1, 2, 3, 0).reshape(cin // 32, 32, 9, cout).permute(0, 2, 3, 1).contiguous())


def fold_bn(bn_weight, bn_bias, mean, var, eps):
    scale = bn_weight / torch.sqrt(var + eps)
    return scale.contiguous(), (bn_bias - mean * scale).contiguous()


LINEAR_ALGO = os.environ.get("AUDIOCAPTION_LINEAR_ALGO", "bf16x3")
_LINEAR_PACKS = {}


def pack_linear_weight_bf16x3_frag(w):
    n, k = w.shape
    return pack_conv_weight_bf16x3_frag(w.reshape(n, k, 1, 1))


def _linear_pack(w):
    import weakref
    hit = _LINEAR_PACKS.get(id(w))
    if hit is not None and hit[0]() is w and hit[1] == w._version and hit[2] == _lib.param_generation():
        return hit[3:]
    for k in [k for k, v in _LINEAR_PACKS.items() if v[0]() is None]:
        del _LINEAR_PACKS[k]
    with torch.no_grad():
        pack = (pack_linear_weight_bf16x3_frag(w.detach().float()), torch.ones(w.shape[0], device=w.device),
                torch.zeros(w.shape[0], device=w.device))
    _LINEAR_PACKS[id(w)] = (weakref.ref(w), w._version, _lib.param_generation()) + pack
    return pack


def linear(x, w, b=None, relu=False, out=None):
    lib = _lib.load()
    M, K = x.shape
    N = w.shape[0]
    if out is None:
        out = torch.empty(M, N, device=x.device, dtype=torch.float32)
    if (LINEAR_ALGO == "bf16x3" and N * K >= 1536 * 512 and K % 32 == 0 and N % 64 == 0 and x.stride(0) == K
            and out.stride(0) == N and w.is_contiguous()):
        wfrag, ones, zeros = _linear_pack(w)
        check(lib.ac_linear_bf16x3(ptr(x), ptr(wfrag), ptr(ones), ptr(b if b is not None else zeros), ptr(out), M, N, K,
                                   1 if relu else 0, stream()), "ac_linear_bf16x3")
        return out
    check(lib.ac_linear(ptr(x), ptr(w), ptr(b), ptr(out), M, N, K, x.stride(0), w.stride(0), out.stride(0),
                        1 if relu else 0, stream()), "ac_linear")
    return out


def gru_pack_whh(whh, hidden):
    lib = _lib.load()
    whh = f32c(_dev(whh))
    out = torch.empty_like(whh)
    check(lib.ac_gru_pack_whh(ptr(whh), ptr(out), hidden, stream()), "ac_gru_pack_whh")
    return out


def gru_layer(gx, whhT, bhh, lens_i32, B, T, hidden):
    lib = _lib.load()
    out = torch.empty(B, T, 2 * hidden, device=gx.device, dtype=torch.float32)
    check(lib.ac_gru_layer(ptr(gx), ptr(whhT), ptr(bhh), ptr(lens_i32), ptr(out), B, T, hidden, stream()),
          "ac_gru_layer")
    return out


def gru_layer_split(gx, whh, bhh, lens_i32, B, T, hidden, workspace=None):
    lib = _lib.load()
    need = lib.ac_gru_split_workspace_bytes(B)
    if workspace is None or workspace.numel() * 8 < need or workspace.device != gx.device:
        workspace = torch.zeros((need + 7) // 8, device=gx.device, dtype=torch.int64)
    out = torch.empty(B, T, 2 * hidden, device=gx.device, dtype=torch.float32)
    check(lib.ac_gru_layer_split(ptr(gx), ptr(whh), ptr(bhh), ptr(lens_i32), ptr(out), None, ptr(workspace), B, T, hidden,
                                 stream()), "ac_gru_layer_split")
    return out, workspace


def gru_split_error(workspace, B):
    return workspace.view(torch.int32)[:1]


def mean_with_lens(x, lens_i32, add_max=False):
    lib = _lib.load()
    B, T, C = x.shape
    out = torch.empty(B, C, device=x.device, dtype=torch.float32)
    check(lib.ac_mean_with_lens(ptr(x), ptr(lens_i32), ptr(out), B, T, C, 1 if add_max else 0, stream()),
          "ac_mean_with_lens")
    return out


def add_layernorm(x, y, w, b, out=None):
    lib = _lib.load()
    rows, d = x.shape
    if out is None:
        out = torch.empty(rows, d, device=x.device, dtype=torch.float32)
    check(lib.ac_add_layernorm(ptr(x), ptr(y), ptr(w), ptr(b), ptr(out), rows, d, x.stride(0),
                               y.stride(0) if y is not None else 0, out.stride(0), stream()), "ac_add_layernorm")
    return out


def dropout_(x, n, p, seed, seed_dev=None):
    lib = _lib.load()
    check(lib.ac_dropout(ptr(x), ptr(x), n, float(p), int(seed), seed_dev, 0, stream()), "ac_dropout")
    return x


def rows_mean_w(x, out, B, Hp, H, W, C):
    lib = _lib.load()
    check(lib.ac_rows_mean_w(ptr(x), ptr(out), B, Hp, H, W, C, stream()), "ac_rows_mean_w")
    return out


def specaug_(x, stripes, fill, B, rows_per_clip, T, n_time=2, n_freq=2):
    lib = _lib.load()
    check(lib.ac_specaug(ptr(x), ptr(stripes), ptr(fill), B, rows_per_clip, T, 64, n_time, n_freq, stream()), "ac_specaug")
    return x


def specaug_stripes(seed, B, T, F=64, time_width=64, time_num=2, freq_width=8, freq_num=2):
    import numpy as np
    rng = np.random.default_rng(int(seed) & 0xFFFFFFFFFFFFFFFF)
    out = np.zeros((B, time_num + freq_num, 2), dtype=np.int32)
    for b in range(B):
        for k in range(time_num):
            d = int(rng.integers(0, time_width))
            out[b, k] = (int(rng.integers(0, T - d)), d)
    for b in range(B):
        for k in range(freq_num):
            d = int(rng.integers(0, freq_width))
            out[b, time_num + k] = (int(rng.integers(0, F - d)), d)
    return out


def pool_avgmax(x, out, B, Hp, H, W, C, ph, Hp_out=0, mean_w=False):
    lib = _lib.load()
    if x.dtype != torch.float32 or out.dtype != torch.float32:
        raise ValueError("pool_avgmax reads and writes f32")
    need_in = B * Hp * W * C
    need_out = B * H * C if mean_w else B * Hp_out * (W // 2) * C
    if x.numel() < need_in or out.numel() < need_out:
        raise ValueError("pool_avgmax: a buffer is smaller than its geometry")
    check(lib.ac_pool_avgmax(ptr(x), ptr(out), B, Hp, H, W, C, ph, Hp_out, 1 if mean_w else 0, stream()), "ac_pool_avgmax")
    return out


def sed_head(x, bias=None, pre=None):
    lib = _lib.load()
    x = f32c(_dev(x))
    rows, C = x.shape
    prob = torch.empty_like(x)
    if pre is not None and (pre.shape != x.shape or pre.dtype != torch.float32 or not pre.is_contiguous()):
        raise ValueError("sed_head: pre must be a contiguous f32 tensor of x's shape")
    check(lib.ac_sed_head(ptr(x), ptr(bias), ptr(pre), ptr(prob), rows, C, stream()), "ac_sed_head")
    return prob


def sed_temporal_tag(prob, frames_num, ratio=4, high=0.75, low=0.25, n_connect=1, time_resolution=0.01, thre=0.5,
                     workspace=None):
    lib = _lib.load()
    prob = f32c(_dev(prob))
    B, S, C = prob.shape
    need = lib.ac_sed_tag_workspace_bytes(B, S, C)
    if workspace is None or workspace.numel() * 4 < need or workspace.device != prob.device:
        workspace = torch.empty((need + 15) // 16, 4, device=prob.device, dtype=torch.int32)
    tags = torch.empty(B, device=prob.device, dtype=torch.int32)
    rule = (ctypes.c_double * 2)(float(time_resolution), float(thre))
    check(lib.ac_sed_temporal_tag(ptr(prob), B, S, C, int(frames_num), int(ratio), float(high), float(low), int(n_connect),
                                  rule, ptr(workspace), workspace.numel() * 4, ptr(tags), stream()), "ac_sed_temporal_tag")
    return tags, workspace
```

include/audiocaption_hip.h:

```cpp
#ifndef AUDIOCAPTION_HIP_H
#define AUDIOCAPTION_HIP_H

#include <stdint.h>

#ifdef __cplusplus
extern "C" {
#endif

#define AC_OK 0
#define AC_ERR_ARG (-1)
#define AC_ERR_LAUNCH (-2)

#define AC_ABI_VERSION 2
int ac_abi_version(void);

int ac_logmel(const float* wav, int B, int L, int n_fft, int hop, const float* window, const float* twiddle,
              const float* melfb, const int* mel_lo, const int* mel_hi, const float* scale, const float* shift,
              float* out, int rows_per_clip, long stride_b, long stride_t, long stride_m, void* stream);

int ac_conv3x3_bn_relu(const float* in, const float* wpk, const float* scale, const float* shift, float* out,
                       int B, int Hp, int H, int W, int Cin, int Cout, int mode, int map_mode, void* stream);
int ac_conv3x3_bn_relu_winograd(const float* in, const float* upk, const float* scale, const float* shift,
                                float* out, int B, int Hp, int H, int W, int Cin, int Cout, int mode,
                                int map_mode, void* stream);
int ac_conv3x3_bn_relu_bf16x3(const float* in, const void* wpk, const float* scale, const float* shift, float* out,
                              int B, int Hp, int H, int W, int Cin, int Cout, int mode, int map_mode, void* stream);
int ac_conv3x3_bn_relu_bf16x3_gw(const float* in, const void* wfrag, const float* scale, const float* shift,
                                 float* out, int B, int Hp, int H, int W, int Cin, int Cout, int mode,
                                 int map_mode, void* stream);
int ac_conv3x3_bn_relu_wino1d(const float* in, const void* wfrag, const float* scale, const float* shift,
                              float* out, int B, int Hp, int H, int W, int Cin, int Cout, int mode,
                              int map_mode, const int* clip_frames, int need_mul, int need_add, void* stream);
int ac_conv3x3_bn_relu_wino1d_drop(const float* in, const void* wfrag, const float* scale, const float* shift,
                                   float* out, int B, int Hp, int H, int W, int Cin, int Cout, int mode, int map_mode,
                                   float drop_p, unsigned long long drop_seed, const unsigned long long* seed_dev,
                                   void* stream);
long ac_conv3x3_wino1d_splitk_floats(int B, int Hp, int W, int Cin, int Cout);
int ac_conv3x3_bn_relu_wino1d_splitk(const float* in, const void* wfrag, const float* scale, const float* shift,
                                     float* out, int B, int Hp, int H, int W, int Cin, int Cout, int mode,
                                     int map_mode, const int* clip_frames, int need_mul, int need_add,
                                     float* workspace, long workspace_floats, void* stream);

long ac_conv3x3_skinny_workspace_floats(int B, int Hp, int W, int Cin, int Cout);
int ac_conv3x3_bn_relu_skinny(const float* in, const void* wfrag, const float* scale, const float* shift, float* out, int B,
                              int Hp, int H, int W, int Cin, int Cout, int mode, float* workspace, long workspace_floats,
                              float drop_p, unsigned long long drop_seed, const unsigned long long* seed_dev, void* stream);

int ac_conv3x3_bn_relu_wino43(const float* in, const void* wfrag, const float* scale, const float* shift, float* out,
                              int B, int Hp, int H, int W, int Cin, int Cout, int mode, int map_mode, int tiles_per_wave,
                              const int* clip_frames, int need_mul, int need_add, void* stream);
int ac_conv3x3_bn_relu_wino43_drop(const float* in, const void* wfrag, const float* scale, const float* shift, float* out,
                                   int B, int Hp, int H, int W, int Cin, int Cout, int mode, int map_mode, float drop_p,
                                   unsigned long long drop_seed, const unsigned long long* seed_dev, void* stream);
long ac_conv3x3_wino43_workgroups(int B, int Hp, int W, int Cout);

int ac_conv3x3_block1_wino43(const float* in1, const float* w1, const float* scale1, const float* shift1,
                             const void* wfrag2, const float* scale2, const float* shift2, float* out, int B, int Hp,
                             int H, const int* clip_frames, int need_mul, int need_add, float drop_p,
                             unsigned long long drop_seed, const unsigned long long* seed_dev, void* stream);
int ac_conv3x3_block1_wino43_mfma(const float* in1, const float* w1, const float* scale1, const float* shift1,
                                  const void* wfrag2, const float* scale2, const float* shift2, float* out, int B, int Hp,
                                  int H, const int* clip_frames, int need_mul, int need_add, float drop_p,
                                  unsigned long long drop_seed, const unsigned long long* seed_dev, void* stream);
int ac_conv3x3_block1_conv2_wino43(const float* in64, const void* wfrag2, const float* scale2, const float* shift2,
                                   float* out, int B, int Hp, int H, void* stream);

int ac_conv3x3_bn_relu_f16x2_gw(const void* in, const void* wfrag, const float* scale, const float* shift,
                                void* out, int B, int Hp, int H, int W, int Cin, int Cout, int mode,
                                int map_mode, int out_f32, unsigned int* overflow_flag, void* stream);
int ac_conv3x3_block1_f16x2(const float* in1, const float* w1, const float* scale1, const float* shift1,
                            const void* wfrag2, const float* scale2, const float* shift2, void* out,
                            int B, int Hp, int H, int W, unsigned int* overflow_flag, void* stream);

int ac_linear_bf16x3(const float* X, const void* wfrag, const float* ones, const float* bias, float* Y,
                     int M, int N, int K, int relu, void* stream);

int ac_conv3x3_first(const float* in, const float* w, const float* scale, const float* shift, float* out,
                     int B, int Hp, int H, int W, void* stream);
int ac_conv3x3_first_f16(const float* in, const float* w, const float* scale, const float* shift, void* out,
                         int B, int Hp, int H, int W, unsigned int* overflow_flag, void* stream);

int ac_conv5x5_first(const float* in, const float* w, const float* scale, const float* shift, float* out,
                     int B, int Hp, int H, void* stream);
int ac_conv5x5_bn_relu_bf16x3(const float* in, const void* wfrag, const float* scale, const float* shift, float* out,
                              int B, int Hp, int H, int W, int Cin, int Cout, int mode, void* stream);
int ac_pack_conv5x5_weight_bf16x3(const float* w, void* wfrag, int Cin, int Cout, void* stream);

int ac_linear(const float* X, const float* W, const float* bias, float* Y, int M, int N, int K, long ldx,
              long ldw, long ldy, int relu, void* stream);

int ac_gru_pack_whh(const float* whh, float* packed, int hidden, void* stream);
int ac_gru_layer(const float* gx, const float* whhT, const float* bhh, const int* lens, float* out, int B,
                 int T, int hidden, void* stream);
long ac_gru_split_workspace_bytes(int B);
int ac_gru_layer_split(const float* gx, const float* whh, const float* bhh, const int* lens, float* out, float* save,
                       void* workspace, int B, int T, int hidden, void* stream);
int ac_mean_with_lens(const float* x, const int* lens, float* out, int B, int T, int C, int add_max,
                      void* stream);

#define AC_MAX_LAYERS 8
typedef struct {
  const float *sa_in_w, *sa_in_b, *sa_out_w, *sa_out_b;
  const float *ca_in_w, *ca_in_b, *ca_out_w, *ca_out_b;
  const float *l1_w, *l1_b, *l2_w, *l2_b;
  const float *n1_w, *n1_b, *n2_w, *n2_b, *n3_w, *n3_b;
} ac_trm_layer;

typedef struct {
  int32_t d_model, nhead, nlayers, dim_ff, vocab, max_pos, attn_emb_dim, reserved;
  const float* emb;
  const float* pe;
  const float* cls_w;
  const float* proj_w;
  const float* proj_b;
  const float* proj_ln_w;
  const float* proj_ln_b;
  const float* step_pk;
  ac_trm_layer layer[AC_MAX_LAYERS];
} ac_trm_weights;

int ac_add_layernorm(const float* x, const float* y, const float* w, const float* b, float* out, int rows,
                     int d, long ldx, long ldy, long ldo, void* stream);

int ac_trm_memory(const ac_trm_weights* w, const float* attn_emb, int R, int Tm, float* memkv, float* tmp,
                  void* stream);

long ac_trm_step_pack_floats(const ac_trm_weights* w);
int ac_trm_pack_step_weights(const ac_trm_weights* w, float* out, void* stream);

long ac_dec_wide_packed_floats(int N, int K);
int ac_dec_wide_pack(const float* W, long ldw, int N, int K, float* out, void* stream);
int ac_dec_wide_gemm(int producer, const float* X, long ldx, const float* Y2, long ldy2, const float* ln_w,
                     const float* ln_b, const int* tok, long tok_stride, int t, const float* emb, const float* pe,
                     float emb_scale, float* xout, long ldxo, const float* Wp, const float* bias, float* Y, long ldy, int M,
                     int N, int K, int relu, int ntb, int split_out, void* stream);

long ac_trm_workspace_floats(const ac_trm_weights* w, int rows, int max_len);

int ac_trm_greedy(const ac_trm_weights* w, const float* memkv, const int* mem_len, int B, int Tm, int max_len,
                  int start_idx, int end_idx, int pad_idx, int64_t* seq, float* logit, float* logprob,
                  float* embed, int* unfinished_cnt, float* ws, void* stream);

int ac_trm_greedy_segments(const ac_trm_weights* w, const float* memkv, const int* mem_len, int B, int segments, int Tm,
                           int max_len, int start_idx, int end_idx, int pad_idx, int64_t* seq, float* logit,
                           float* logprob, float* embed, int* unfinished_cnt, float* ws, void* stream);

long ac_trm_cluster_pack_floats(const ac_trm_weights* w);
int ac_trm_cluster_pack(const ac_trm_weights* w, float* out, void* stream);
long ac_trm_cluster_workspace_bytes(int B);
int ac_trm_greedy_cluster(const ac_trm_weights* w, const float* cluster_pk, const float* memkv, const int* mem_len, int B,
                          int Tm, int max_len, int start_idx, int end_idx, int pad_idx, int64_t* seq, float* logit,
                          float* logprob, float* embed, int* unfinished_cnt, void* workspace, int early_stop, void* stream);

#define AC_SAMPLE_PLAIN 0
#define AC_SAMPLE_TOPK 1
#define AC_SAMPLE_TOPP 2
#define AC_SAMPLE_GUMBEL 3

int ac_sample_rows(const float* logit, long ld, int rows, int V, int method, int k, float top_p, float temp,
                   const uint64_t* seed_dev, int step, int* word_out, float* logprob_out, void* stream);

int ac_trm_sample(const ac_trm_weights* w, const float* memkv, const int* mem_len, int B, int Tm, int max_len,
                  int start_idx, int end_idx, int pad_idx, int64_t* seq, float* logit, float* logprob,
                  float* embed, int* unfinished_cnt, float* ws, int method, int k, float top_p, float temp,
                  const uint64_t* seed_dev, void* stream);

int ac_trm_sample_multi(const ac_trm_weights* w, const float* memkv, const int* mem_len, int B, int samples_per_clip,
                        int Tm, int max_len, int start_idx, int end_idx, int pad_idx, int64_t* seq, float* logit,
                        float* logprob, float* embed, int* unfinished_cnt, float* ws, int method, int k, float top_p,
                        float temp, const uint64_t* seed_dev, void* stream);

int ac_trm_forward_tokens(const ac_trm_weights* w, const float* memkv, const int* mem_len, int N, int Tm,
                          const int* tokens, const unsigned char* key_mask, int T, float* embed, float* logit,
                          float* ws, void* stream);

int ac_trm_beam_step(const ac_trm_weights* w, const float* memkv, const int* mem_len, int B, int beam, int Tm,
                     int max_len, int t, float temp, const int* tokens, const unsigned char* key_mask,
                     const float* cum_logprob, float* top_val, int* top_idx, float* ws, void* stream);
int ac_trm_beam_update(const float* top_val, const int* top_idx, const int* tokens_in, int* tokens_out,
                       unsigned char* key_mask_out, float* cum_logprob, int* active, int* done_count, int* done_seq,
                       float* done_score, int* src_row, int* n_active, int B, int beam, int V, int max_len, int t,
                       int end_idx, int pad_idx, int done_capacity, void* stream);
int ac_trm_beam_reorder(const ac_trm_weights* w, int R, int max_len, int t, const int* src_row, float* ws,
                        void* stream);

int ac_trm_beam_update_all(const float* top_val, const int* top_idx, const int* tokens_in, int* tokens_out,
                           unsigned char* key_mask_out, float* cum_logprob, int* active, int* done_count, int* done_seq,
                           float* done_score, int* src_row, int* n_active, int B, int beam, int V, int max_len, int t,
                           int end_idx, int pad_idx, int done_capacity, void* stream);

typedef struct {
  const float* kwp;
  const float* ln_w;
  const float* ln_b;
  int32_t row_div;
} ac_trm_keyword;
int ac_trm_kw_greedy_segments(const ac_trm_weights* w, const ac_trm_keyword* kw, const float* memkv, const int* mem_len,
                              int B, int segments, int Tm, int max_len, int start_idx, int end_idx, int pad_idx,
                              int64_t* seq, float* logit, float* logprob, float* embed, int* unfinished_cnt, float* ws,
                              void* stream);
int ac_trm_kw_sample(const ac_trm_weights* w, const ac_trm_keyword* kw, const float* memkv, const int* mem_len, int B, int Tm,
                     int max_len, int start_idx, int end_idx, int pad_idx, int64_t* seq, float* logit, float* logprob,
                     float* embed, int* unfinished_cnt, float* ws, int method, int k, float top_p, float temp,
                     const uint64_t* seed_dev, void* stream);
int ac_trm_kw_forward_tokens(const ac_trm_weights* w, const ac_trm_keyword* kw, const float* memkv, const int* mem_len, int N,
                             int Tm, const int* tokens, const unsigned char* key_mask, int T, float* embed, float* logit,
                             float* ws, void* stream);
int ac_trm_kw_beam_step(const ac_trm_weights* w, const ac_trm_keyword* kw, const float* memkv, const int* mem_len, int B,
                        int beam, int Tm, int max_len, int t, float temp, const int* tokens, const unsigned char* key_mask,
                        const float* cum_logprob, float* top_val, int* top_idx, float* ws, void* stream);
int ac_trm_kw_embed_qkv(const ac_trm_weights* w, const ac_trm_keyword* kw, int R, int row_div, int t, const int* tokens,
                        long tok_stride, float* xout, float* qkv, void* stream);

#define AC_ENS_MAX 8
int ac_trm_step_logits(const ac_trm_weights* w, const float* memkv, const int* mem_len, int R, int row_div, int Tm,
                       int max_len, int t, const int* tokens, const unsigned char* key_mask, int cache_set,
                       float* logit, long ldl, float* embed, long ld_embed, float* ws, void* stream);

int ac_ens_greedy_pick(const float* const* logits, int n_models, long ld, int rows, int V, int t, int max_len,
                       int end_idx, int pad_idx, int64_t* seq, float* logprob, int* tokens, unsigned char* key_mask,
                       int* unfinished, int* unfinished_cnt, void* stream);
int ac_ens_sample_pick(const float* const* logits, int n_models, long ld, int rows, int V, int method, int k,
                       float top_p, float temp, const uint64_t* seed_dev, int t, int max_len, int end_idx, int pad_idx,
                       int64_t* seq, float* logprob, int* tokens, unsigned char* key_mask, int* unfinished,
                       int* unfinished_cnt, int* word_out, void* stream);
int ac_ens_beam_step_select(const float* const* logits, int n_models, long ld, int B, int beam, int V, int t, float temp,
                            const float* cum_logprob, float* top_val, int* top_idx, float* scratch, void* stream);

#define AC_GROUP_BEAM_MAX_GROUPS 8
int ac_group_beam_select(const float* logit, long ldl, int B, int bdash, int V, int lt, float temp,
                         float diversity_lambda, const float* cum, const int* const* prev_tok, int n_prev, long tok_ld,
                         float* top_val, int* top_idx, float* scratch, void* stream);

#define AC_SEARCH_GREEDY (-1)
typedef struct {
  float repetition_penalty;
  int32_t no_repeat_ngram, min_length, end_idx, n_bad;
  const int32_t* bad_words;
} ac_logit_rules;
int ac_logit_rules_apply(const float* logit, long ld_in, float* out, long ld_out, int rows, int V, const int* tokens,
                         long ld_tok, int t, const ac_logit_rules* rules, void* stream);
int ac_trm_search_rules(const ac_trm_weights* w, const float* memkv, const int* mem_len, int R, int row_div, int Tm,
                        int max_len, int start_idx, int end_idx, int pad_idx, int64_t* seq, float* logit, float* logprob,
                        float* embed, int* unfinished_cnt, float* ws, int method, int k, float top_p, float temp,
                        const uint64_t* seed_dev, const ac_logit_rules* rules, float* plane, long ld_plane, void* stream);
int ac_trm_beam_step_rules(const ac_trm_weights* w, const float* memkv, const int* mem_len, int B, int beam, int Tm,
                           int max_len, int t, float temp, const int* tokens, const unsigned char* key_mask,
                           const float* cum_logprob, float* top_val, int* top_idx, float* ws,
                           const ac_logit_rules* rules, float* plane, void* stream);

typedef struct {
  int32_t emb_dim, d_model, attn_size, attn_emb_dim, fc_emb_dim, vocab, n_tags;
  int32_t variant;
  const float* emb;
  const float* temb;
  const float* w_ih;
  const float* w_hh;
  const float* b_ih;
  const float* b_hh;
  const float* attn_w;
  const float* attn_b;
  const float* attn_v;
  const float* fc_w;
  const float* fc_b;
  const float* ctx_w;
  const float* ctx_b;
  const float* cls_w;
  const float* cls_b;
} ac_bah_weights;

int ac_bah_memory_cond(const ac_bah_weights* w, const float* attn_emb, const float* cond, int B, int R, int Tm, int max_len,
                       float* ws, void* stream);
long ac_bah_workspace_floats(const ac_bah_weights* w, int B, int R, int Tm, int max_len);
int ac_bah_memory(const ac_bah_weights* w, const float* attn_emb, const float* fc_emb, int B, int R, int Tm, int max_len,
                  float* ws, void* stream);
int ac_bah_step_logits(const ac_bah_weights* w, const float* attn_emb, const int* mem_len, int B, int R, int row_div,
                       int Tm, int max_len, const float* state_in, const int* words, long word_stride, const int* tags,
                       float* state_out, float* embed, long ld_embed, float* logit, long ldl, float* attn_weight,
                       long attn_row_stride, long attn_frame_stride, float* ws, void* stream);
int ac_bah_greedy(const ac_bah_weights* w, const float* attn_emb, const int* mem_len, const int* tags, int B, int Tm,
                  int max_len, int start_idx, int end_idx, int pad_idx, int64_t* seq, float* logit, float* logprob,
                  float* embed, float* attn_weight, float* state, int* unfinished_cnt, float* ws, void* stream);
int ac_bah_sample(const ac_bah_weights* w, const float* attn_emb, const int* mem_len, const int* tags, int B, int Tm,
                  int max_len, int start_idx, int end_idx, int pad_idx, int64_t* seq, float* logit, float* logprob,
                  float* embed, float* attn_weight, float* state, int* unfinished_cnt, float* ws, int method, int k,
                  float top_p, float temp, const uint64_t* seed_dev, void* stream);
int ac_bah_beam_gather(const int* src_row, const int* active_before, const float* state_new, float* state_next,
                       const float* step_weight, const float* hist_in, float* hist_out, int B, int beam, int d, int Tm,
                       int max_len, int t, void* stream);

long ac_bah_train_workspace_floats(const ac_bah_weights* w, int B, int Tm, int T);
int ac_bah_train_forward(const ac_bah_weights* w, const float* attn_emb, const float* fc_emb, const int* mem_len,
                         const long long* cap, long cap_ld, const int* use_cap, const int* tags, int B, int Tm, int T,
                         int start_idx, float drop_p, unsigned long long drop_seed, const unsigned long long* seed_dev,
                         int64_t* seq, float* logit, float* logprob, float* embed, float* attn_weight, float* state,
                         float* ws, void* stream);
int ac_bah_train_rollout(const ac_bah_weights* w, const float* attn_emb, const float* fc_emb, const int* mem_len,
                         const int* tags, int B, int Tm, int T, int start_idx, int end_idx, float temp,
                         const uint64_t* sample_seed_dev, const int* forced, long forced_ld, float drop_p,
                         unsigned long long drop_seed, const unsigned long long* seed_dev, int* seq, int* scratch,
                         float* logit, float* logprob, float* embed, float* attn_weight, float* state, float* ws,
                         void* stream);
typedef struct {
  float *emb, *temb, *w_ih, *w_hh, *b_ih, *b_hh, *attn_w, *attn_b, *attn_v, *fc_w, *fc_b, *ctx_w, *ctx_b, *cls_w, *cls_b;
} ac_bah_grads;
int ac_bah_train_backward(const ac_bah_weights* w, const ac_bah_grads* g, const float* attn_emb, const float* fc_emb,
                          const int* mem_len, const float* dlogit, int B, int Tm, int T, float drop_p,
                          unsigned long long drop_seed, const unsigned long long* seed_dev, float* d_attn_emb,
                          float* d_fc_emb, float* ws, void* stream);
int ac_bah_train_forward_cond(const ac_bah_weights* w, const float* attn_emb, const float* cond, const int* mem_len,
                              const long long* cap, long cap_ld, const int* use_cap, int B, int Tm, int T, int start_idx,
                              float drop_p, unsigned long long drop_seed, const unsigned long long* seed_dev, int64_t* seq,
                              float* logit, float* logprob, float* embed, float* attn_weight, float* state, float* ws,
                              void* stream);
int ac_bah_train_backward_cond(const ac_bah_weights* w, const ac_bah_grads* g, const float* attn_emb, const float* cond,
                               const int* mem_len, const float* dlogit, int B, int Tm, int T, float drop_p,
                               unsigned long long drop_seed, const unsigned long long* seed_dev, float* d_attn_emb,
                               float* d_fc_emb, float* ws, void* stream);
int ac_bah_mean_lens_bwd(const float* d_fc_emb, const int* lens, float* d_attn_emb, int B, int Tm, int A, int F,
                         void* stream);

int ac_specificity_loss(const float* logit, const float* word_spec, const int* tgt_len, const float* cond, int N, int T,
                        int V, int mean_reduce, float* row_s, float* row_lse, float* diff, float* loss, void* stream);
int ac_specificity_loss_bwd(const float* logit, const float* word_spec, const int* tgt_len, const float* row_s,
                            const float* row_lse, const float* diff, const float* g_dev, int N, int T, int V,
                            int mean_reduce, float* dlogit, void* stream);

int ac_pool_avgmax(const float* in, float* out, int B, int Hp, int H, int W, int C, int ph, int Hp_out, int mean_w,
                   void* stream);
int ac_sed_head(const float* x, const float* bias, float* pre, float* prob, long rows, int C, void* stream);
long ac_sed_tag_workspace_bytes(int B, int S, int C);
int ac_sed_temporal_tag(const float* prob, int B, int S, int C, int frames_num, int ratio, float high, float low,
                        int n_connect, const double* rule, void* workspace, long workspace_bytes, int* tags, void* stream);


int ac_gemm(const float* A, long sam, long sak, const float* B, long sbk, long sbn, float* C, long ldc, int M, int N,
            int K, const float* bias, int relu, float beta, int splitk, float drop_p, unsigned long long drop_seed,
            const unsigned long long* seed_dev, long row0, const float* a_scale, int a_rows, void* stream);
int ac_gemm_bf16x3(const float* A, long sam, long sak, const float* B, long sbk, long sbn, float* C, long ldc, int M,
                   int N, int K, const float* bias, int relu, float beta, int splitk, float drop_p,
                   unsigned long long drop_seed, const unsigned long long* seed_dev, long row0, const float* a_scale,
                   int a_rows, void* stream);
int ac_dropout(const float* x, float* y, long n, float p, unsigned long long seed, const unsigned long long* seed_dev,
               long idx0, void* stream);
int ac_mask_pos_scale(float* g, const float* h, long n, float scale, void* stream);
int ac_build_prefix(const long long* cap, int cap_ld, const int* seq, int seq_ld, const int* use_cap, int t,
                    int start_idx, int* word, long row0, int N, int L, void* stream);
int ac_embed_fwd(const float* emb, const float* pe, const int* word, const int* pos, float* x, long row0, long rows,
                 int d, float pa, unsigned long long seed_a, float pb, unsigned long long seed_b,
                 const unsigned long long* seed_dev, void* stream);
int ac_embed_bwd(const float* dx, const int* word, float* demb, long rows, int d, float pa, unsigned long long seed_a,
                 float pb, unsigned long long seed_b, const unsigned long long* seed_dev, void* stream);
int ac_kw_embed_fwd(const float* emb, const float* pe, const int* word, const int* pos, const int* clip, const float* kwp,
                    const float* gamma, const float* beta, float* pre, float* x, long row0, long rows, int d, float pa,
                    unsigned long long seed_a, float pb, unsigned long long seed_b, const unsigned long long* seed_dev,
                    float eps, void* stream);
int ac_kw_embed_bwd(const float* dx, const int* word, const int* clip, const float* pre, const float* gamma, float* dgamma,
                    float* dbeta, float* dkwp, float* demb, long rows, int d, float pa, unsigned long long seed_a, float pb,
                    unsigned long long seed_b, const unsigned long long* seed_dev, float eps, void* stream);
int ac_dropadd_ln_fwd(const float* x, const float* res, const float* gamma, const float* beta, float* pre, float* y,
                      long row0, long rows, long xmod, int d, float p, unsigned long long seed,
                      const unsigned long long* seed_dev, float eps, void* stream);
int ac_dropadd_ln_bwd(const float* dy, const float* pre, const float* gamma, float* dx, float* dres, int accumulate,
                      const float* relu_src, long relu_mod, float* dgamma, float* dbeta, long rows, int d, float p,
                      unsigned long long seed, const unsigned long long* seed_dev, float eps, void* stream);
int ac_attn_seq_fwd(const float* q, long ldq, const float* k, long ldk, const float* v, long ldv, float* o, long ldo,
                    float* P, int pl, int ptk, const int* qrow0, const int* qlen, const int* krow0, const int* klen,
                    const int* kvalid, const int* word, int pad_idx, int causal, int seq0, int nseq, int nhead,
                    int head_dim, int lmax, int tkmax, float drop_p, unsigned long long seed,
                    const unsigned long long* seed_dev, void* stream);
int ac_attn_seq_bwd(const float* q, long ldq, const float* k, long ldk, const float* v, long ldv, const float* P, int pl,
                    int ptk, const float* dout, long lddo, float* dq, long lddq, float* dk, long lddk, float* dv,
                    long lddv, const int* qrow0, const int* qlen, const int* krow0, const int* klen, int seq0, int nseq,
                    int nhead, int head_dim, int lmax, int tkmax, float drop_p, unsigned long long seed,
                    const unsigned long long* seed_dev, void* stream);
int ac_attn_self_bwd_tiled(const float* q, long ldq, const float* k, long ldk, const float* v, long ldv, const float* P,
                           int pl, int ptk, const float* dout, long lddo, float* dq, long lddq, float* dk, long lddk,
                           float* dv, long lddv, const int* qrow0, const int* qlen, const int* krow0, const int* klen,
                           int seq0, int nseq, int nhead, int head_dim, int lmax, int tkmax, float drop_p,
                           unsigned long long seed, const unsigned long long* seed_dev, float* d_ws, void* stream);
int ac_gather_rows(const float* src, const int* index, float* dst, long nrows, int C, void* stream);
int ac_scatter_add_rows(const float* src, const int* index, float* dst, long nrows, int C, void* stream);
int ac_specaug(float* x, const int* stripes, const float* fill, int B, int rows_per_clip, int T, int F, int n_time,
               int n_freq, void* stream);
int ac_sum_replicas(const float* x, float* out, long n, int reps, void* stream);
int ac_rows_mean_w(const float* x, float* out, int B, int Hp, int H, int W, int C, void* stream);
int ac_transpose(const float* src, float* dst, int batch, int rows, int cols, void* stream);
int ac_colsum(const float* x, long ld, float* out, long M, int N, void* stream);
int ac_argmax_rows(const float* logit, long ld, int rows, int V, int* out, long out_ld, void* stream);
int ac_label_smoothing_loss(const float* logit, const long long* tgt, long tgt_ld, const int* tgt_len, int N, int T, int V,
                            float smoothing, float inv_count, float* row_loss, float* loss, float* dlogit, float gscale,
                            const float* gscale_dev, void* stream);
int ac_scst_pick(const float* logit, long ld, int N, int V, float temp, const uint64_t* seed_dev, int t, int end_idx,
                 const int* forced, long forced_ld, int* done, int* drawn, int* seq, long seq_ld, float* logprob, long lp_ld,
                 void* stream);
int ac_scst_loss(const float* logit, const int* seq, long seq_ld, const float* reward, float temp, int end_idx, int N, int T,
                 int V, float* row_loss, float* loss, float* dlogit, const float* gscale_dev, void* stream);
#define AC_SCST_MAX_ROLLOUTS 8
#define AC_SCST_BASELINE_GREEDY 0
#define AC_SCST_BASELINE_MEAN 1
int ac_scst_group_reward(const float* scores, int K, int N, int mode, const float* greedy_scores, float* reward,
                         void* stream);
int ac_kd_loss(const float* logit, const float* tchr_logit, const long long* tgt, long tgt_ld, const int* tgt_len, int N,
               int T, int V, float smoothing, float temp, float sup_weight, float inv_count, float* row_sup, float* row_kd,
               float* loss, float* dlogit, float gscale, const float* gscale_dev, void* stream);
#define AC_ENC_KD_CONTRA 1
#define AC_ENC_KD_MSE 2
#define AC_ENC_KD_L2NORM 4
long ac_enc_kd_workspace_floats(int B, int D);
int ac_enc_kd_loss(const float* s, long ld_s, const float* t, long ld_t, int B, int D, int kind, const float* logit_scale,
                   float* loss, float* ds, float* dt, float* dscale, float gscale, const float* gscale_dev, float* ws,
                   void* stream);
#define AC_CIDER_MAX_SETS 4
#define AC_CIDER_MAX_HYP_WORDS 1024
#define AC_CIDER_MAX_REF_WORDS 1024
long ac_cider_workspace_bytes(long ref_words, int sentences, int keys, int sets);
int ac_cider_scores(const int* const* hyp, int sets, long hyp_ld, int N, int T, int start_idx, int end_idx,
                    const int* canon, int vocab_size, int n_words, const int* ref_words, long total_words,
                    const int* sent_off, int sentences, int max_ref_words, const int* key_off, int keys,
                    const int* row_key, const int* first_row, int order, float sigma, void* workspace,
                    long workspace_bytes, float* scores, float* reward, void* stream);
long ac_capmetrics_workspace_bytes(int keys, int sets);
int ac_bleu_scores(const int* const* hyp, int sets, long hyp_ld, int N, int T, int start_idx, int end_idx,
                   const int* canon, int vocab_size, const int* ref_words, long total_words, const int* sent_off,
                   int sentences, int max_ref_words, const int* key_off, int keys, const int* row_key,
                   const int* first_row, int order, void* workspace, long workspace_bytes, int* stats, double* scores,
                   double* corpus, void* stream);
int ac_rouge_l_scores(const int* const* hyp, int sets, long hyp_ld, int N, int T, int start_idx, int end_idx,
                      const int* canon, int vocab_size, const int* ref_words, long total_words, const int* sent_off,
                      int sentences, int max_ref_words, const int* key_off, int keys, const int* row_key,
                      const int* first_row, void* workspace, long workspace_bytes, int* lcs, double* scores, double* mean,
                      void* stream);
long ac_diversity_workspace_bytes(int N, int T);
int ac_diversity_scores(const int* hyp, long hyp_ld, int N, int T, int start_idx, int end_idx, const int* canon,
                        int vocab_size, void* workspace, long workspace_bytes, int* stats, int* sent_distinct, int* totals,
                        double* self_bleu, double* summary, void* stream);
long ac_diversity_group_workspace_bytes(int N, int T, int G);
int ac_diversity_group_scores(const int* hyp, long hyp_ld, int N, int T, int start_idx, int end_idx, const int* canon,
                              int vocab_size, const int* group_off, int G, void* workspace, long workspace_bytes,
                              int* stats, int* sent_distinct, double* self_bleu, double* mbleu, int* group_totals,
                              double* group_mean, double* summary, void* stream);
int ac_gru_layer_train(const float* gx, const float* whhT, const float* bhh, const int* lens, float* out, float* save,
                       int B, int T, int hidden, void* stream);
int ac_gru_layer_bwd(const float* dout, const float* out, const float* save, const float* whh, const int* lens,
                     float* dgx, float* dgh, float* hprev, int B, int T, int hidden, void* stream);
int ac_swa_update(float* avg, const float* p, long n, int n_averaged, void* stream);
int ac_grad_sumsq(const float* g, long n, float* norm_state, void* stream);
int ac_clip_coef(float* norm_state, float max_norm, float grad_div, void* stream);
int ac_scale_by_coef(float* x, long n, const float* norm_state, void* stream);
int ac_adam_step(float* p, const float* g, float* m, float* v, long n, const float* norm_state, float lr, float beta1,
                 float beta2, float eps, float weight_decay, int step, const int* step_dev, void* stream);
int ac_adam_commit(int* step_dev, const float* norm_state, void* stream);


int ac_pointwise_conv(const float* x, const float* w, const float* bias, float* y, long M, int N, int K, int act, float beta,
                      const float* gate, int gate_rows, void* stream);
int ac_top_db_clamp(float* x, long n, float top_db, float* scratch, int scratch_floats, void* stream);
int ac_effnet_stem(const float* x, const float* w, const float* scale, const float* shift, float* y, int B, int T, int F,
                   int C, int pad_before, int pad_after, void* stream);
int ac_effnet_depthwise(const float* x, const float* w, const float* scale, const float* shift, float* y, float* pool,
                        float pool_scale, int B, int T, int F, int C, int k, int stride, int pad_before, int pad_after,
                        void* stream);
int ac_effnet_se_gate(const float* pool, float inv_count, const float* w1, const float* b1, const float* w2,
                      const float* b2, float* gate, int B, int C, int S, void* stream);
long ac_pw_gemm_packed_bytes(int N, int K);
int ac_pw_gemm_pack(const float* w, void* wfrag, int N, int K, void* stream);
int ac_pw_gemm_bf16x3(const float* x, const void* wfrag, const float* bias, float* y, long M, int N, int K, int act,
                      float beta, const float* gate, int gate_rows, void* stream);
int ac_pw_gemm_bf16x3_ex(const float* x, long ldx, const void* wfrag, const float* bias, float* y, long ldy, long M, int N,
                         int K, int act, float beta, const float* gate, int gate_rows, float drop_p,
                         unsigned long long drop_seed, const unsigned long long* seed_dev, long row0, void* stream);
int ac_pw_gemm_pack_strided(const float* w, long s_n, long s_k, void* wfrag, int N, int K, void* stream);
int ac_pw_gemm_pack_table(const void* table, int count, void* stream);
int ac_effnet_se_gate_t(const float* pool, float inv_count, const float* w1, const float* b1, const float* w2t,
                        const float* b2, float* gate, int B, int C, int S, void* stream);
int ac_effnet_expand_depthwise(const float* x, const float* we, const float* be, const float* wd, const float* scale,
                               const float* shift, float* y, float* pool, float pool_scale, int B, int T, int F, int Cin,
                               int Cmid, int k, int stride, int pad_before, int pad_after, void* stream);

int ac_ingest_resample(const void* src, int src_half, const long* src_off, const float* kernel, const int* tap_lo,
                       const int* tap_hi, float* out, const int* out_len, const int* out_start, int B, int lmax, int orig,
                       int new_, int width, void* stream);

int ac_htsat_patch_embed(const float* x, int B, int T, const float* w, const float* bias,
                         const float* ln_w, const float* ln_b, float* out, int C, void* stream);
int ac_swin_window_attn(const float* qkv, const float* bias, float* out, int B, int H, int W, int C, int heads, int shift,
                        void* stream);
int ac_swin_patch_merge(const float* x, const float* ln_w, const float* ln_b, float* out, int B, int H, int W, int C,
                        void* stream);
int ac_htsat_pool(const float* x, float* attn, float* fc, int B, int Hh, int Ww, int C, int fbins, void* stream);
int ac_htsat_token_mean(const float* x, float* out, int B, int N, int C, void* stream);
int ac_gelu(const float* x, float* y, long n, void* stream);

int ac_mfma_bf16_probe(float* out, int blocks, int iters, void* stream);

int ac_placement_probe(int* out, int blocks, int threads, int spin_ticks, void* stream);

int ac_stream_create_cu_mask(int first_cu, int n_cus, void** out);
int ac_stream_destroy(void* stream);

#ifdef __cplusplus
}
#endif
#endif
```

Before: 15590.

## Add F(6,3) row-sextet Winograd conv path for block 2-3 layers

Generalizes the F(4,3) Winograd MFMA conv kernel with a row-count template parameter and adds an F(6,3) variant that produces six output rows per tile from eight transformed input rows. It also adds host-side weight packing for the 8-point transform and routes selected inference layers to the new kernel when the grid is large enough: W=32 with 128->128 channels and W=16 with 128->256. The aim is fewer multiplies per output and less input-transform and LDS traffic per output row. In exchange it uses larger transforms with less stable constants (bf16x3 accuracy risk), more registers and LDS, and a different ring depth.

```diff
diff --git a/audiocaption_amd/_lib.py b/audiocaption_amd/_lib.py
--- a/audiocaption_amd/_lib.py
+++ b/audiocaption_amd/_lib.py
@@ -67,6 +67,8 @@
     "ac_conv3x3_bn_relu_wino43": (_I, [_P, _P, _P, _P, _P, _I, _I, _I, _I, _I, _I, _I, _I, _I, _P, _I, _I, _P]),
     "ac_conv3x3_bn_relu_wino43_drop": (_I, [_P, _P, _P, _P, _P, _I, _I, _I, _I, _I, _I, _I, _I, _F, _U64, _P, _P]),
     "ac_conv3x3_wino43_workgroups": (_L, [_I, _I, _I, _I]),
+    "ac_conv3x3_bn_relu_wino63": (_I, [_P, _P, _P, _P, _P, _I, _I, _I, _I, _I, _I, _I, _I, _I, _P, _I, _I, _P]),
+    "ac_conv3x3_bn_relu_wino63_drop": (_I, [_P, _P, _P, _P, _P, _I, _I, _I, _I, _I, _I, _I, _I, _F, _U64, _P, _P]),
     "ac_conv3x3_block1_wino43": (_I, [_P, _P, _P, _P, _P, _P, _P, _P, _I, _I, _I, _P, _I, _I, _F, _U64, _P, _P]),
     "ac_conv3x3_block1_wino43_mfma": (_I, [_P, _P, _P, _P, _P, _P, _P, _P, _I, _I, _I, _P, _I, _I, _F, _U64, _P, _P]),
     "ac_conv3x3_block1_conv2_wino43": (_I, [_P, _P, _P, _P, _P, _I, _I, _I, _P]),
diff --git a/audiocaption_amd/cnn_encoder.py b/audiocaption_amd/cnn_encoder.py
--- a/audiocaption_amd/cnn_encoder.py
+++ b/audiocaption_amd/cnn_encoder.py
@@ -38,7 +38,7 @@
 
 
 def _conv_wino1d(x, w, scale, shift, out, B, Hp, H, W, Cin, Cout, mode, need=None, dropout=None, workspace=None,
-                 overflow=None, cold=False):
+                 overflow=None, cold=False, train=False):
     if not wino1d_covers(Cout):
         K.conv3x3_bn_relu_bf16x3_gw(x, w, scale, shift, out, B, Hp, H, W, Cin, Cout, mode)
         if dropout is not None:
@@ -74,14 +74,34 @@
     return W in (32, 16, 8, 4, 2) and cout % 128 == 0
 
 
+def _sextet_layers(default):
+    env = os.environ.get("AUDIOCAPTION_W63_LAYERS")
+    if env is None:
+        return dict(default)
+    return {tuple(v[:3]): v[3] for v in (tuple(int(t) for t in item.split("x")) for item in env.split(",") if item.strip())}
+
+
+SEXTET_LAYERS = _sextet_layers({(32, 128, 128): 2, (16, 128, 256): 1})
+SEXTET_MIN_WORKGROUPS = int(os.environ.get("AUDIOCAPTION_W63_MIN_WG", "1024"))
+
+
+def sextet_route(B, Hp, W, Cin, Cout):
+    return (W, Cin, Cout) in SEXTET_LAYERS and Hp % 4 == 0 and K.wino43_workgroups(B, Hp, W, Cout) >= SEXTET_MIN_WORKGROUPS
+
+
 class Wino43Pack(NamedTuple):
     f23: torch.Tensor
     f43: torch.Tensor = None
     skinny: "_LazyPack" = None
+    f63: torch.Tensor = None
 
 
 def _conv_wino43(x, w, scale, shift, out, B, Hp, H, W, Cin, Cout, mode, need=None, dropout=None, workspace=None,
-                 overflow=None, cold=False):
+                 overflow=None, cold=False, train=False):
+    if w.f63 is not None and need is None and dropout is None and not train and mode != 2 \
+            and sextet_route(B, Hp, W, Cin, Cout):
+        return K.conv3x3_bn_relu_wino63(x, w.f63, scale, shift, out, B, Hp, H, W, Cin, Cout, mode,
+                                        tiles_per_wave=SEXTET_LAYERS[(W, Cin, Cout)])
     if w.f43 is not None and (mode != 1 if W == 2 else mode != 2) and Hp % 4 == 0 \
             and K.wino43_workgroups(B, Hp, W, Cout) >= W43_MIN_WORKGROUPS:
         return K.conv3x3_bn_relu_wino43(x, w.f43, scale, shift, out, B, Hp, H, W, Cin, Cout, mode, need=need, dropout=dropout)
@@ -148,7 +168,7 @@
 
 def _plain(kernel, takes_overflow=False):
     def launch(x, w, scale, shift, out, B, Hp, H, W, Cin, Cout, mode, need=None, dropout=None, workspace=None, overflow=None,
-               cold=False):
+               cold=False, train=False):
         if need is not None or dropout is not None:
             raise ValueError("this conv tier has neither dead-row skipping nor a dropout epilogue")
         if takes_overflow:
@@ -168,7 +188,8 @@
 def _pack_wino43(w, b, weight):
     return Wino43Pack(_pack_wino1d(w, b, weight)[0],
                       K.pack_conv_weight_wino43_frag(w) if wino43_covers(64 >> b, w.shape[0]) else None,
-                      _LazyPack(weight) if b >= 4 else None), None
+                      _LazyPack(weight) if b >= 4 else None,
+                      K.pack_conv_weight_wino63_frag(w) if (64 >> b, w.shape[1], w.shape[0]) in SEXTET_LAYERS else None), None
 
 
 def _block1_wino43(x0, conv1, conv2, f43, out, B, Hp, H, need, dropout, overflow):
@@ -357,7 +378,7 @@
         if specaug is not None:
             K.specaug_(x0, specaug, pk["bn0"][1], B, Hp[0], T)
         return self.conv_stack(x0, B, H, Hp, pk, algo, dropout, overflow=overflow, clip_frames=clip_frames,
-                               block6_f23=block6_f23)
+                               block6_f23=block6_f23, train=train or dropout is not None)
 
     def effective_algo(self, algo=None, train=False, min_frames=None):
         algo = algo or self.conv_algo
@@ -367,13 +388,13 @@
         return algo
 
     def conv_stack(self, x0, B, H, Hp, pk, algo, dropout=None, blocks=None, overflow=None, clip_frames=None,
-                   block6_f23=False):
+                   block6_f23=False, train=False):
         dev = x0.device
         tiers = [conv_tier(algo)] * 5 + [pk["block6"]]
         full = self._buf("full", B * Hp[0] * 64 * 64, dev, tiers[0].act)
         pooled = self._buf("pooled", B * Hp[1] * 32 * 64, dev, tiers[0].act)
         W = 64
-        offer = {"workspace": None, "overflow": overflow, "cold": dropout is not None}
+        offer = {"workspace": None, "overflow": overflow, "cold": dropout is not None, "train": train}
         if os.environ.get("AUDIOCAPTION_W1_SPLITK", "1") != "0":
             offer["workspace"] = lambda n: self._buf("w1_splitk", n, dev)
         fuse1 = os.environ.get("AUDIOCAPTION_FUSE_BLOCK1", "1") != "0"
diff --git a/audiocaption_amd/csrc/ac_wino43.h b/audiocaption_amd/csrc/ac_wino43.h
--- a/audiocaption_amd/csrc/ac_wino43.h
+++ b/audiocaption_amd/csrc/ac_wino43.h
@@ -49,6 +49,33 @@
   y[3] = fmaxf(fmaf(__builtin_fmaf(8.f, d34, d12) + m5, sc, sh), 0.f);
 }
 
+__device__ __forceinline__ f32x4 w6_transform(int pos, const f32x4& d0, const f32x4& d1, const f32x4& d2, const f32x4& d3,
+                                              const f32x4& d4, const f32x4& d5, const f32x4& d6, const f32x4& d7) {
+  if (pos == 0) return vfma(5.25f, d4 - d2, d0 - d6);
+  if (pos == 7) return vfma(5.25f, d3 - d5, d7 - d1);
+  if (pos == 1 || pos == 2) {
+    const f32x4 te = vfma(-4.25f, d4, d2 + d6), to = vfma(-4.25f, d3, d1 + d5);
+    return pos == 1 ? te + to : te - to;
+  }
+  if (pos == 3 || pos == 4) {
+    const f32x4 te = vfma(0.25f, d2, vfma(-1.25f, d4, d6)), to = vfma(2.f, d5, vfma(-2.5f, d3, 0.5f * d1));
+    return pos == 3 ? te + to : te - to;
+  }
+  const f32x4 te = vfma(4.f, d2, vfma(-5.f, d4, d6)), to = vfma(2.f, d1, vfma(-2.5f, d3, 0.5f * d5));
+  return pos == 5 ? te + to : te - to;
+}
+
+__device__ __forceinline__ void w6_outputs(float m0, float m1, float m2, float m3, float m4, float m5, float m6, float m7,
+                                           float sc, float sh, float (&y)[6]) {
+  const float s12 = m1 + m2, d12 = m1 - m2, s34 = m3 + m4, d34 = m3 - m4, s56 = m5 + m6, d56 = m5 - m6;
+  y[0] = fmaxf(fmaf(((m0 + s12) + s34) + s56, sc, sh), 0.f);
+  y[1] = fmaxf(fmaf(__builtin_fmaf(0.5f, d56, __builtin_fmaf(2.f, d34, d12)), sc, sh), 0.f);
+  y[2] = fmaxf(fmaf(__builtin_fmaf(0.25f, s56, __builtin_fmaf(4.f, s34, s12)), sc, sh), 0.f);
+  y[3] = fmaxf(fmaf(__builtin_fmaf(0.125f, d56, __builtin_fmaf(8.f, d34, d12)), sc, sh), 0.f);
+  y[4] = fmaxf(fmaf(__builtin_fmaf(0.0625f, s56, __builtin_fmaf(16.f, s34, s12)), sc, sh), 0.f);
+  y[5] = fmaxf(fmaf(__builtin_fmaf(0.03125f, d56, __builtin_fmaf(32.f, d34, d12)) + m7, sc, sh), 0.f);
+}
+
 struct FastDiv4 {
   int d;
   float inv;
diff --git a/audiocaption_amd/csrc/conv3x3_wino43.hip b/audiocaption_amd/csrc/conv3x3_wino43.hip
--- a/audiocaption_amd/csrc/conv3x3_wino43.hip
+++ b/audiocaption_amd/csrc/conv3x3_wino43.hip
@@ -14,6 +14,9 @@
 
 #ifndef W4_RING
 #define W4_RING 9
+#endif
+#ifndef W6_RING
+#define W6_RING 8
 #endif
 #ifndef W4_PRO2
 #define W4_PRO2 1
@@ -34,6 +37,7 @@
 
 constexpr int KS = 16;
 constexpr int W4_OUT_TILE = 4 * 32 * 144;
+constexpr int W6_OUT_TILE = 3 * 32 * 144;
 
 struct W4Params {
   const float* in;
@@ -80,10 +84,13 @@
   return true;
 }
 
-template <int TC, int MW>
+template <int TC, int MW, int R = 4>
 struct W4Geom {
   static_assert(TC == 32 || TC == 16 || TC == 8 || TC == 4 || TC == 2, "full-width blocks of 32, 16, 8, 4 or 2 mel columns");
   static_assert(MW == 1 || MW == 2, "one or two MFMA tiles per wave");
+  static_assert(R == 4 || (R == 6 && TC >= 8), "row quads, or row sextets in conv blocks 2-4");
+  static constexpr int NP = R + 2;
+  static constexpr int NG = 3 * NP;
   static constexpr bool COLT = TC == 2;
   static_assert(!COLT || MW == 2, "column tiles: one tile per column");
   static constexpr int QT = COLT ? 32 : 32 / TC;
@@ -92,17 +99,18 @@
   static constexpr int COLP = COLT ? 32 : TC == 32 ? (PQ | 1) : TC == 16 ? (PQ % 4 == 2 ? PQ : PQ + 2) : (PQ % 8 == 4 ? PQ : PQ + 4);
   static constexpr int HALF = ((LCOLS * COLP * 16 + 127) / 128) * 128 + 64;
   static constexpr int PLANE = 2 * HALF;
-  static constexpr int VBUF = 12 * PLANE;
+  static constexpr int VBUF = 2 * NP * PLANE;
   static constexpr int NITEM = PQ * TC * 4;
   static_assert(NITEM == 256 || NITEM == 128, "one item per thread (MW = 1: per thread of waves 0 and 1)");
-  static constexpr int NPIECE = 6;
+  static constexpr int NPIECE = NP;
+  static constexpr int OUT_TILE = R == 4 ? W4_OUT_TILE : W6_OUT_TILE;
 };
 
-template <int MODE, int TC, int MW>
+template <int MODE, int TC, int MW, int R = 4>
 __global__ __launch_bounds__(256, MW == 1 ? 2 : 1) void conv3x3_w4_kernel(W4Params p) {
-  using G = W4Geom<TC, MW>;
+  using G = W4Geom<TC, MW, R>;
   constexpr int QT = G::QT, PQ = G::PQ, COLP = G::COLP, HALF = G::HALF, PLANE = G::PLANE, VBUF = G::VBUF;
-  constexpr int NPIECE = G::NPIECE;
+  constexpr int NPIECE = G::NPIECE, NP = G::NP, NG = G::NG;
   extern __shared__ __attribute__((aligned(128))) unsigned char dsm_raw[];
   const int tid = threadIdx.x;
   const int lane = tid & 63;
@@ -128,16 +136,16 @@
                       : (unsigned)(half * HALF + ((i % TC) * COLP + m * QT + i / TC) * 16);
   }
 
-  f32x16 acc[6][MW];
-#pragma unroll
-  for (int q = 0; q < 6; ++q)
+  f32x16 acc[NP][MW];
+#pragma unroll
+  for (int q = 0; q < NP; ++q)
 #pragma unroll
     for (int m = 0; m < MW; ++m)
 #pragma unroll
       for (int r = 0; r < 16; ++r) acc[q][m][r] = 0.f;
 
-  const int row0 = 4 * quad0;
-  const bool live = w4_rows_live(row0, 4 * PQ, p.rows_total, p.Hp, p.H, p.clip_frames, p.need_mul, p.need_add);
+  const int row0 = R * quad0;
+  const bool live = w4_rows_live(row0, R * PQ, p.rows_total, p.Hp, p.H, p.clip_frames, p.need_mul, p.need_add);
   const bool all_pad = !live;
   const int nstep = p.Cin / KS;
   if (!all_pad) {
@@ -150,11 +158,11 @@
     const int NT32 = p.Cout >> 5;
     const unsigned g_bytes = (unsigned)NT32 * 2048u;
     const __amdgpu_buffer_rsrc_t rw = __builtin_amdgcn_make_buffer_rsrc(
-        (void*)p.wpk, 0, (int)((unsigned)nstep * 18u * g_bytes), 0x00020000);
+        (void*)p.wpk, 0, (int)((unsigned)nstep * (unsigned)NG * g_bytes), 0x00020000);
     const unsigned wvoff = (unsigned)((n_tile * 4 + wave) * 2048 + lane * 16);
     auto w_load = [&](int s, int gi, bf16x8 (&w)[2]) {
       if (W4_KO & 1) { if (s | gi) return; }
-      const unsigned soff = (unsigned)(s * 18 + gi) * g_bytes;
+      const unsigned soff = (unsigned)(s * NG + gi) * g_bytes;
       w[0] = __builtin_bit_cast(bf16x8, __builtin_amdgcn_raw_buffer_load_b128(rw, wvoff, soff, 0));
       w[1] = __builtin_bit_cast(bf16x8, __builtin_amdgcn_raw_buffer_load_b128(rw, wvoff + 1024u, soff, 0));
     };
@@ -165,7 +173,7 @@
     {
       auto item = [&](int it, unsigned& vb, unsigned& lofs) {
         const int cq = it & 3, rest = it >> 2, quad = rest % PQ, c = rest / PQ;
-        vb = (unsigned)(((4 * quad - first) * p.W + c) * p.Cin * 4 + cq * 16);
+        vb = (unsigned)(((R * quad - first) * p.W + c) * p.Cin * 4 + cq * 16);
         lofs = (unsigned)((cq >> 1) * HALF + ((c + (G::COLT ? 0 : 1)) * COLP + quad) * 16 + (cq & 1) * 8);
       };
       item(stager ? tid : 0, vbA, lofsA);
@@ -174,12 +182,12 @@
     auto run = [&]() {
       constexpr bool PAIR = W4_ROWPAIR && MW == 2;
       static_assert(!PAIR || W4_PRO2, "the paired form starts from the two-step prologue");
-      f32x4 preA[6], rwp[PAIR ? 6 : 1];
+      f32x4 preA[NP], rwp[PAIR ? NP : 1];
       auto rows_request_pair = [&](int s) {
         if (W4_KO & 8) { if (s > 1) return; }
         const unsigned cs = (unsigned)(s * KS * 4);
 #pragma unroll
-        for (int r = 0; r < 6; ++r) {
+        for (int r = 0; r < NP; ++r) {
           preA[r] = __builtin_bit_cast(f32x4, __builtin_amdgcn_raw_buffer_load_b128(rin, vbA + cs + (unsigned)r * row_bytes, 0, 0));
           rwp[PAIR ? r : 0] = __builtin_bit_cast(f32x4, __builtin_amdgcn_raw_buffer_load_b128(rin, vbA + cs + (unsigned)(KS * 4) + (unsigned)r * row_bytes, 0, 0));
         }
@@ -189,7 +197,7 @@
         if (!stager) return;
         const unsigned cs = (unsigned)(s * KS * 4);
 #pragma unroll
-        for (int r = 0; r < 6; ++r)
+        for (int r = 0; r < NP; ++r)
           preA[r] = __builtin_bit_cast(f32x4, __builtin_amdgcn_raw_buffer_load_b128(rin, vbA + cs + (unsigned)r * row_bytes, 0, 0));
       };
       auto store_piece = [&](unsigned char* buf, unsigned lofs, int pos, const f32x4 v) {
@@ -199,20 +207,27 @@
         *(u32x2*)dst = hi;
         *(u32x2*)(dst + PLANE) = lo;
       };
+      auto transform = [](int k, const f32x4* d, auto PRESENT_) {
+        constexpr bool PRESENT = decltype(PRESENT_)::value;
+        if constexpr (R == 4)
+          return w4_transform(k, d[0], d[PRESENT ? 1 : 0], d[PRESENT ? 2 : 0], d[PRESENT ? 3 : 0], d[PRESENT ? 4 : 0], d[PRESENT ? 5 : 0]);
+        else
+          return w6_transform(k, d[0], d[PRESENT ? 1 : 0], d[PRESENT ? 2 : 0], d[PRESENT ? 3 : 0], d[PRESENT ? 4 : 0], d[PRESENT ? 5 : 0],
+                              d[PRESENT ? 6 : 0], d[PRESENT ? 7 : 0]);
+      };
       auto commit_piece_set1 = [&](unsigned char* buf, int k) {
         if (W4_KO & 4) return;
-        store_piece(buf, lofsA, k, w4_transform(k, rwp[0], rwp[PAIR ? 1 : 0], rwp[PAIR ? 2 : 0], rwp[PAIR ? 3 : 0],
-                                                rwp[PAIR ? 4 : 0], rwp[PAIR ? 5 : 0]));
+        store_piece(buf, lofsA, k, transform(k, rwp, std::integral_constant<bool, PAIR>{}));
       };
       auto commit_piece = [&](unsigned char* buf, int k) {
         if (W4_KO & 4) return;
         if (!stager) return;
-        store_piece(buf, lofsA, k, w4_transform(k, preA[0], preA[1], preA[2], preA[3], preA[4], preA[5]));
+        store_piece(buf, lofsA, k, transform(k, preA, std::true_type{}));
       };
       auto tap_valid = [](int m, int kx) { return !G::COLT || (m + kx - 1 >= 0 && m + kx - 1 <= 1); };
       auto a_load = [&](const unsigned char* buf, int gi, bf16x8 (&a)[MW][2]) {
         if (W4_KO & 2) { if (gi) return; }
-        const int kx = gi / 6, q = gi % 6;
+        const int kx = gi / NP, q = gi % NP;
         const unsigned char* vh = buf + (2 * q) * PLANE;
         const int koff = (G::COLT ? kx - 1 : kx) * COLP * 16;
 #pragma unroll
@@ -224,24 +239,25 @@
       };
 
       {
-        constexpr int NZ = G::COLT ? 0 : 2 * 12 * 2 * 2 * COLP;
+        constexpr int PH = 4 * NP;
+        constexpr int NZ = G::COLT ? 0 : 2 * PH * 2 * COLP;
         const f32x4 z = {0.f, 0.f, 0.f, 0.f};
         for (int i = tid; i < NZ; i += 256) {
-          const int slot = i % COLP, col = (i / COLP) & 1, hh = (i / (2 * COLP)) % 24, b = i / (48 * COLP);
+          const int slot = i % COLP, col = (i / COLP) & 1, hh = (i / (2 * COLP)) % PH, b = i / (2 * PH * COLP);
           *(f32x4*)(sV + b * VBUF + hh * HALF + ((col ? TC + 1 : 0) * COLP + slot) * 16) = z;
         }
       }
-      constexpr int RING = MW == 1 ? 6 : W4_RING, AH = RING - 1, NA = W4_ADEPTH + 1, LASTG = 17 - W4_ADEPTH;
-      static_assert(18 % RING == 0 && 18 % NA == 0 && NPIECE <= LASTG, "ring positions are static; staging ends before the barrier");
+      constexpr int RING = MW == 1 ? 6 : R == 4 ? W4_RING : W6_RING, AH = RING - 1, NA = W4_ADEPTH + 1, LASTG = NG - 1 - W4_ADEPTH;
+      static_assert(NG % RING == 0 && NG % NA == 0 && NPIECE <= LASTG, "ring positions are static; staging ends before the barrier");
       bf16x8 wr[RING][2];
 #if W4_PRO2
-      f32x4 pre2[6];
+      f32x4 pre2[NP];
       if (PAIR) rows_request_pair(0);
       else rows_request(0);
       if (MW == 2 && !PAIR) {
         const unsigned cs = (unsigned)(KS * 4);
 #pragma unroll
-        for (int r = 0; r < 6; ++r)
+        for (int r = 0; r < NP; ++r)
           pre2[r] = __builtin_bit_cast(f32x4, __builtin_amdgcn_raw_buffer_load_b128(rin, vbA + cs + (unsigned)r * row_bytes, 0, 0));
       }
 #pragma unroll
@@ -251,7 +267,7 @@
       if (PAIR) {
       } else if (MW == 2) {
 #pragma unroll
-        for (int r = 0; r < 6; ++r) preA[r] = pre2[r];
+        for (int r = 0; r < NP; ++r) preA[r] = pre2[r];
       } else {
         rows_request(1);
       }
@@ -274,14 +290,14 @@
         const unsigned char* cur = sV + (s & 1) * VBUF;
         unsigned char* nxt = sV + ((s + 1) & 1) * VBUF;
 #pragma unroll
-        for (int gi = 0; gi < 18; ++gi) {
-          const int q = gi % 6;
-          if (gi + W4_ADEPTH < 18) a_load(cur, gi + W4_ADEPTH, af[(gi + W4_ADEPTH) % NA]);
-          else if (MORE) a_load(nxt, gi + W4_ADEPTH - 18, af[(gi + W4_ADEPTH) % NA]);
-          if (gi + AH < 18) w_load(s, gi + AH, wr[(gi + AH) % RING]);
-          else if (MORE) w_load(s + 1, gi + AH - 18, wr[(gi + AH) % RING]);
+        for (int gi = 0; gi < NG; ++gi) {
+          const int q = gi % NP;
+          if (gi + W4_ADEPTH < NG) a_load(cur, gi + W4_ADEPTH, af[(gi + W4_ADEPTH) % NA]);
+          else if (MORE) a_load(nxt, gi + W4_ADEPTH - NG, af[(gi + W4_ADEPTH) % NA]);
+          if (gi + AH < NG) w_load(s, gi + AH, wr[(gi + AH) % RING]);
+          else if (MORE) w_load(s + 1, gi + AH - NG, wr[(gi + AH) % RING]);
           if (!(W4_KO & 32)) {
-            const int kxg = gi / 6;
+            const int kxg = gi / NP;
 #pragma unroll
             for (int m = 0; m < MW; ++m)
               if (tap_valid(m, kxg))
@@ -297,7 +313,7 @@
           } else {
 #pragma unroll
             for (int m = 0; m < MW; ++m)
-              if (tap_valid(m, gi / 6))
+              if (tap_valid(m, gi / NP))
                 asm volatile("" :: "v"(af[gi % NA][m][0]), "v"(af[gi % NA][m][1]), "v"(wr[gi % RING][0]), "v"(wr[gi % RING][1]));
           }
           if (MORE) {
@@ -371,46 +387,58 @@
   for (int m = 0; m < MW; ++m) {
     const int col = G::COLT ? m : pi % TC;
     const int qg = quad0 + (G::COLT ? pi : m * QT + pi / TC);
-    const int gr = 4 * qg;
-    f32x4 y[4][4];
+    const int gr = R * qg;
+    f32x4 y[4][R];
 #pragma unroll
     for (int g = 0; g < 4; ++g)
 #pragma unroll
       for (int e = 0; e < 4; ++e) {
         const int r = 4 * g + e;
-        float yy[4];
-        w4_outputs(acc[0][m][r], acc[1][m][r], acc[2][m][r], acc[3][m][r], acc[4][m][r], acc[5][m][r], sc4[g][e], sh4[g][e], yy);
-#pragma unroll
-        for (int j = 0; j < 4; ++j) y[g][j][e] = yy[j];
-      }
-    unsigned char* wt = dsm_raw + wave * W4_OUT_TILE;
+        float yy[R];
+        if constexpr (R == 4)
+          w4_outputs(acc[0][m][r], acc[1][m][r], acc[2][m][r], acc[3][m][r], acc[4][m][r], acc[5][m][r], sc4[g][e], sh4[g][e], yy);
+        else
+          w6_outputs(acc[0][m][r], acc[1][m][r], acc[2][m][r], acc[3][m][r], acc[4][m][r], acc[5][m][r], acc[NP - 2][m][r],
+                     acc[NP - 1][m][r], sc4[g][e], sh4[g][e], yy);
+#pragma unroll
+        for (int j = 0; j < R; ++j) y[g][j][e] = yy[j];
+      }
+    unsigned char* wt = dsm_raw + wave * G::OUT_TILE;
     constexpr int PITCH = 144;
     const int P8 = lane >> 3, q8 = lane & 7;
     if (MODE == MODE_FULL) {
+      constexpr int RH = R == 4 ? 4 : 3;
       const int h = by_hp.mod(gr);
 #pragma unroll
-      for (int j = 0; j < 4; ++j)
-#pragma unroll
-        for (int g = 0; g < 4; ++g)
-          *(f32x4*)(wt + (j * 32 + pi) * PITCH + (2 * g + half) * 16) = h + j < p.H ? y[g][j] : zero4;
-#pragma unroll
-      for (int k = 0; k < 4; ++k) {
-        const int px = 8 * k + P8;
-        const int pcol = G::COLT ? m : px % TC;
-        const int pgr = 4 * (quad0 + (G::COLT ? px : m * QT + px / TC));
-#pragma unroll
-        for (int j = 0; j < 4; ++j) {
-          f32x4 v = *(const f32x4*)(wt + (j * 32 + px) * PITCH + q8 * 16);
-          const size_t oi = ((size_t)(pgr + j) * p.W + pcol) * p.Cout + n_tile * 128 + wave * 32 + 4 * q8;
-          if (p.drop.thresh != 0) {
-#pragma unroll
-            for (int e = 0; e < 4; ++e) v[e] *= p.drop.mask(oi + e);
+      for (int j0 = 0; j0 < R; j0 += RH) {
+#pragma unroll
+        for (int j = 0; j < RH; ++j) {
+          const bool inside = (R == 4 ? h + j : by_hp.mod(gr + j0 + j)) < p.H;
+#pragma unroll
+          for (int g = 0; g < 4; ++g)
+            *(f32x4*)(wt + (j * 32 + pi) * PITCH + (2 * g + half) * 16) = inside ? y[g][j0 + j] : zero4;
+        }
+#pragma unroll
+        for (int k = 0; k < 4; ++k) {
+          const int px = 8 * k + P8;
+          const int pcol = G::COLT ? m : px % TC;
+          const int pgr = R * (quad0 + (G::COLT ? px : m * QT + px / TC));
+#pragma unroll
+          for (int j = 0; j < RH; ++j) {
+            f32x4 v = *(const f32x4*)(wt + (j * 32 + px) * PITCH + q8 * 16);
+            const size_t oi = ((size_t)(pgr + j0 + j) * p.W + pcol) * p.Cout + n_tile * 128 + wave * 32 + 4 * q8;
+            if (p.drop.thresh != 0) {
+#pragma unroll
+              for (int e = 0; e < 4; ++e) v[e] *= p.drop.mask(oi + e);
+            }
+            if ((R == 4 ? pgr : pgr + j0 + j) < p.rows_total && !(W4_KO & 64)) *(f32x4*)(p.out + oi) = v;
           }
-          if (pgr < p.rows_total && !(W4_KO & 64)) *(f32x4*)(p.out + oi) = v;
         }
       }
     } else {
-      const bool valid = by_hp_out.mod(2 * qg) + (col & 1) < p.H_out;
+      constexpr int PR = R / 2;
+      const int prow = PR * qg + (col & 1);
+      const bool valid = R == 4 ? by_hp_out.mod(2 * qg) + (col & 1) < p.H_out : by_hp_out.mod(prow) < p.H_out;
 #pragma unroll
       for (int g = 0; g < 4; ++g) {
         const f32x4 t0 = y[g][0] + y[g][1], t1 = y[g][2] + y[g][3];
@@ -427,12 +455,37 @@
         const int px = 8 * k + P8;
         const int pcol = px % TC, pqg = quad0 + m * QT + px / TC;
         f32x4 o = *(const f32x4*)(wt + px * PITCH + q8 * 16);
-        const size_t oi = ((size_t)(2 * pqg + (pcol & 1)) * p.W_out + (pcol >> 1)) * p.Cout + n_tile * 128 + wave * 32 + 4 * q8;
+        const int orow = PR * pqg + (pcol & 1);
+        const size_t oi = ((size_t)orow * p.W_out + (pcol >> 1)) * p.Cout + n_tile * 128 + wave * 32 + 4 * q8;
         if (p.drop.thresh != 0) {
 #pragma unroll
           for (int e = 0; e < 4; ++e) o[e] *= p.drop.mask(oi + e);
         }
-        if (4 * pqg < p.rows_total && !(W4_KO & 64)) *(f32x4*)(p.out + oi) = o;
+        if ((R == 4 ? 4 * pqg : 2 * orow) < p.rows_total && !(W4_KO & 64)) *(f32x4*)(p.out + oi) = o;
+      }
+      if constexpr (R == 6) {
+        const bool valid2 = by_hp_out.mod(PR * qg + 2) < p.H_out;
+#pragma unroll
+        for (int g = 0; g < 4; ++g) {
+          const f32x4 t2 = y[g][4] + y[g][5];
+          f32x4 o;
+#pragma unroll
+          for (int e = 0; e < 4; ++e) o[e] = 0.25f * (t2[e] + dpp_mov<DPP_QUAD_XOR1>(t2[e]));
+          if (!(col & 1)) *(f32x4*)(wt + (pi >> 1) * PITCH + (2 * g + half) * 16) = valid2 ? o : zero4;
+        }
+#pragma unroll
+        for (int k = 0; k < 2; ++k) {
+          const int px = 2 * (8 * k + P8);
+          const int pcol = px % TC, pqg = quad0 + m * QT + px / TC;
+          f32x4 o = *(const f32x4*)(wt + (px >> 1) * PITCH + q8 * 16);
+          const int orow = PR * pqg + 2;
+          const size_t oi = ((size_t)orow * p.W_out + (pcol >> 1)) * p.Cout + n_tile * 128 + wave * 32 + 4 * q8;
+          if (p.drop.thresh != 0) {
+#pragma unroll
+            for (int e = 0; e < 4; ++e) o[e] *= p.drop.mask(oi + e);
+          }
+          if (2 * orow < p.rows_total && !(W4_KO & 64)) *(f32x4*)(p.out + oi) = o;
+        }
       }
     }
   }
@@ -450,27 +503,27 @@
 #endif
 }
 
-template <int MODE, int TC, int MW>
+template <int MODE, int TC, int MW, int R = 4>
 int launch_w4(W4Params p, hipStream_t s) {
-  using G = W4Geom<TC, MW>;
-  const int quads = p.rows_total / 4;
+  using G = W4Geom<TC, MW, R>;
+  const int quads = (p.rows_total + R - 1) / R;
   p.MT = (quads + G::PQ - 1) / G::PQ;
   unsigned grid;
   if (p.map_mode == 2) grid = (unsigned)(((p.MT + 7) / 8) * 8 * p.NT);
   else if (p.map_mode == 3 || p.map_mode == 4) grid = (unsigned)(((p.MT + 8 / p.NT - 1) / (8 / p.NT)) * 8);
   else grid = (unsigned)(p.MT * p.NT);
-  constexpr size_t lds = (size_t)2 * G::VBUF > (size_t)4 * W4_OUT_TILE ? (size_t)2 * G::VBUF : (size_t)4 * W4_OUT_TILE;
-  static_assert(lds <= 160 * 1024, "V planes exceed the LDS");
+  constexpr size_t lds = (size_t)2 * G::VBUF > (size_t)4 * G::OUT_TILE ? (size_t)2 * G::VBUF : (size_t)4 * G::OUT_TILE;
+  static_assert(lds <= 160 * 1024 && (MW == 2 || lds <= 80 * 1024), "V planes exceed the LDS (half-size form: of two workgroups)");
   static AcLdsAttr lds_attr;
-  if (ac_allow_lds((const void*)conv3x3_w4_kernel<MODE, TC, MW>, 160 * 1024, &lds_attr) != AC_OK) return AC_ERR_LAUNCH;
-  hipLaunchKernelGGL((conv3x3_w4_kernel<MODE, TC, MW>), dim3(grid), dim3(256), lds, s, p);
+  if (ac_allow_lds((const void*)conv3x3_w4_kernel<MODE, TC, MW, R>, 160 * 1024, &lds_attr) != AC_OK) return AC_ERR_LAUNCH;
+  hipLaunchKernelGGL((conv3x3_w4_kernel<MODE, TC, MW, R>), dim3(grid), dim3(256), lds, s, p);
   return ac_check_launch();
 }
 
-template <int MODE, int TC>
+template <int MODE, int TC, int R = 4>
 int launch_w4_mw(const W4Params& p, int mw, hipStream_t s) {
-  if (mw == 1) return launch_w4<MODE, TC, 1>(p, s);
-  return launch_w4<MODE, TC, 2>(p, s);
+  if (mw == 1) return launch_w4<MODE, TC, 1, R>(p, s);
+  return launch_w4<MODE, TC, 2, R>(p, s);
 }
 
 }
@@ -482,14 +535,15 @@
 
 static int w4_dispatch(const float* in, const void* wfrag, const float* scale, const float* shift, float* out, int B, int Hp,
                        int H, int W, int Cin, int Cout, int mode, int map_mode, int mw, const int* clip_frames, int need_mul,
-                       int need_add, void* stream, Drop drop) {
+                       int need_add, void* stream, Drop drop, int rows = 4) {
   if (!in || !wfrag || !scale || !shift || !out) return AC_ERR_ARG;
+  if (rows == 6 && !(W == 32 || W == 16 || W == 8)) return AC_ERR_ARG;
   if (B <= 0 || Hp <= H || (Hp & 3) || !(W == 32 || W == 16 || W == 8 || W == 4 || W == 2) || Cin % 32 || Cin < 32 || Cout % 128)
     return AC_ERR_ARG;
   if (W == 2 ? (mode != MODE_FULL && mode != MODE_MEANW) : (mode != MODE_FULL && mode != MODE_POOL)) return AC_ERR_ARG;
   if (mode == MODE_MEANW && drop.thresh != 0) return AC_ERR_ARG;
   if ((unsigned long long)B * Hp >= (1ull << 23)) return AC_ERR_ARG;
-  if ((unsigned long long)(Cin / 16) * 18 * (Cout / 32) * 2048 >= (1ull << 31)) return AC_ERR_ARG;
+  if ((unsigned long long)(Cin / 16) * (3 * (rows + 2)) * (Cout / 32) * 2048 >= (1ull << 31)) return AC_ERR_ARG;
   W4Params p;
   p.in = in; p.wpk = wfrag; p.scale = scale; p.shift = shift; p.out = out;
   p.rows_total = B * Hp; p.Hp = Hp; p.H = H; p.W = W; p.Cin = Cin; p.Cout = Cout;
@@ -515,6 +569,13 @@
   }
   if (W == 2) mw = 2;
   hipStream_t s = (hipStream_t)stream;
+  if (rows == 6) {
+#define W6_CASE(TCV)                                                                     \
+  if (W == TCV) return mode == MODE_FULL ? launch_w4_mw<MODE_FULL, TCV, 6>(p, mw, s) : launch_w4_mw<MODE_POOL, TCV, 6>(p, mw, s);
+    W6_CASE(32) W6_CASE(16) W6_CASE(8)
+#undef W6_CASE
+    return AC_ERR_ARG;
+  }
 #define W4_CASE(TCV)                                                                     \
   if (W == TCV) return mode == MODE_FULL ? launch_w4_mw<MODE_FULL, TCV>(p, mw, s) : launch_w4_mw<MODE_POOL, TCV>(p, mw, s);
   W4_CASE(32) W4_CASE(16) W4_CASE(8) W4_CASE(4)
@@ -552,3 +613,20 @@
   if (B <= 0 || Hp <= 0 || (Hp & 3) || !(W == 32 || W == 16 || W == 8 || W == 4 || W == 2) || Cout % 128) return 0;
   return w4_grid(B * Hp, W, Cout, 2);
 }
+
+extern "C" int ac_conv3x3_bn_relu_wino63(const float* in, const void* wfrag, const float* scale, const float* shift,
+                                         float* out, int B, int Hp, int H, int W, int Cin, int Cout, int mode,
+                                         int map_mode, int tiles_per_wave, const int* clip_frames, int need_mul,
+                                         int need_add, void* stream) {
+  return w4_dispatch(in, wfrag, scale, shift, out, B, Hp, H, W, Cin, Cout, mode, map_mode, tiles_per_wave, clip_frames,
+                     need_mul, need_add, stream, make_drop(0.f, 0, nullptr), 6);
+}
+
+extern "C" int ac_conv3x3_bn_relu_wino63_drop(const float* in, const void* wfrag, const float* scale, const float* shift,
+                                              float* out, int B, int Hp, int H, int W, int Cin, int Cout, int mode,
+                                              int map_mode, float drop_p, unsigned long long drop_seed,
+                                              const unsigned long long* seed_dev, void* stream) {
+  if (!(drop_p >= 0.f) || drop_p >= 1.f) return AC_ERR_ARG;
+  return w4_dispatch(in, wfrag, scale, shift, out, B, Hp, H, W, Cin, Cout, mode, map_mode, 0, nullptr, 0, 0, stream,
+                     make_drop(drop_p, drop_seed, seed_dev), 6);
+}
diff --git a/audiocaption_amd/kernels.py b/audiocaption_amd/kernels.py
--- a/audiocaption_amd/kernels.py
+++ b/audiocaption_amd/kernels.py
@@ -224,6 +224,24 @@
     return out
 
 
+def conv3x3_bn_relu_wino63(x, wfrag, scale, shift, out, B, Hp, H, W, Cin, Cout, mode, map_mode=-1, need=None, dropout=None,
+                           tiles_per_wave=0):
+    lib = _lib.load()
+    cf, mul, add = need if need is not None else (None, 0, 0)
+    if dropout is not None and cf is not None:
+        raise ValueError("conv3x3_bn_relu_wino63: dropout and dead-row skipping are not combined")
+    with _observed("wino43", B, Hp, H, W, Cin, Cout, mode):
+        if dropout is not None:
+            check(lib.ac_conv3x3_bn_relu_wino63_drop(ptr(x), ptr(wfrag), ptr(scale), ptr(shift), ptr(out), B, Hp, H, W, Cin,
+                                                     Cout, mode, map_mode, float(dropout[0]), int(dropout[1]), dropout[2],
+                                                     stream()), "ac_conv3x3_bn_relu_wino63_drop")
+        else:
+            check(lib.ac_conv3x3_bn_relu_wino63(ptr(x), ptr(wfrag), ptr(scale), ptr(shift), ptr(out), B, Hp, H, W, Cin, Cout,
+                                                mode, map_mode, int(tiles_per_wave), ptr(cf), int(mul), int(add), stream()),
+                  "ac_conv3x3_bn_relu_wino63")
+    return out
+
+
 def skinny_workspace_floats(B, Hp, W, Cin, Cout):
     return int(_lib.load().ac_conv3x3_skinny_workspace_floats(B, Hp, W, Cin, Cout))
 
@@ -307,6 +325,26 @@
     def lay(t):
         t = t.permute(1, 2, 0).reshape(cin // 16, 2, 8, 18, cout // 32, 32)
         return t.permute(0, 3, 4, 1, 5, 2).reshape(cin // 16, 18, cout // 32, 64, 8)
+
+    return torch.stack([lay(hi), lay(lo)], dim=3).contiguous()
+
+
+WINO63_G = ((1, 0, 0), (-2 / 9, -2 / 9, -2 / 9), (-2 / 9, 2 / 9, -2 / 9), (1 / 90, 1 / 45, 2 / 45), (1 / 90, -1 / 45, 2 / 45),
+            (32 / 45, 16 / 45, 8 / 45), (32 / 45, -16 / 45, 8 / 45), (0, 0, 1))
+
+
+def pack_conv_weight_wino63_frag(w):
+    cout, cin = w.shape[0], w.shape[1]
+    g = w.double()
+    G = WINO63_G
+    u = torch.stack([G[p][0] * g[:, :, 0] + G[p][1] * g[:, :, 1] + G[p][2] * g[:, :, 2] for p in range(8)], dim=3)
+    u = u.reshape(cout, cin, 24)
+    hi = u.to(torch.bfloat16)
+    lo = (u - hi.double()).to(torch.bfloat16)
+
+    def lay(t):
+        t = t.permute(1, 2, 0).reshape(cin // 16, 2, 8, 24, cout // 32, 32)
+        return t.permute(0, 3, 4, 1, 5, 2).reshape(cin // 16, 24, cout // 32, 64, 8)
 
     return torch.stack([lay(hi), lay(lo)], dim=3).contiguous()
 
diff --git a/include/audiocaption_hip.h b/include/audiocaption_hip.h
--- a/include/audiocaption_hip.h
+++ b/include/audiocaption_hip.h
@@ -53,6 +53,13 @@
                                    int B, int Hp, int H, int W, int Cin, int Cout, int mode, int map_mode, float drop_p,
                                    unsigned long long drop_seed, const unsigned long long* seed_dev, void* stream);
 long ac_conv3x3_wino43_workgroups(int B, int Hp, int W, int Cout);
+
+int ac_conv3x3_bn_relu_wino63(const float* in, const void* wfrag, const float* scale, const float* shift, float* out,
+                              int B, int Hp, int H, int W, int Cin, int Cout, int mode, int map_mode, int tiles_per_wave,
+                              const int* clip_frames, int need_mul, int need_add, void* stream);
+int ac_conv3x3_bn_relu_wino63_drop(const float* in, const void* wfrag, const float* scale, const float* shift, float* out,
+                                   int B, int Hp, int H, int W, int Cin, int Cout, int mode, int map_mode, float drop_p,
+                                   unsigned long long drop_seed, const unsigned long long* seed_dev, void* stream);
 
 int ac_conv3x3_block1_wino43(const float* in1, const float* w1, const float* scale1, const float* shift1,
                              const void* wfrag2, const float* scale2, const float* shift2, float* out, int B, int Hp,
```

Result: faster. 15800 (median of 6 runs) (+1.3%).
